# parsaeskandar/pangenome-index

Measured on AMD Instinct MI355X. Metric: find_mems reads/sec (150 bp batch), higher is better.
Workload: dtype u64

## Files before the change

pangenome-index_amd/csrc/pgx_batch.hip:

```cpp
#include <memory>
#include <string>
#include <thread>

#include "pgx_runtime_internal.hpp"

struct pgx_chunk { uint64_t r0, r1, slot_base, slots; };

struct pgx_batch {
    pgx_index *h = nullptr;
    pgx_device_image *dimg = nullptr;
    int device = 0;
    hipStream_t own = nullptr;
    hipStream_t side = nullptr;
    hipEvent_t ev_side[2] = {nullptr, nullptr};
    bool class_valid = false, class_ok = false;
    uint64_t side_reads_est = 0;
    uint64_t n_reads = 0, read_bytes = 0;
    HostBuf h_off[2];
    int h_off_cur = 0;
    const uint64_t *h_offsets() const { return h_off[h_off_cur].as<uint64_t>(); }
    std::vector<pgx_chunk> chunks;
    bool plan_valid = false, slot_off_valid = false;
    uint64_t slot_off_min_len = 0;
    uint64_t plan_min_len = 0, plan_budget = 0;
// ... 243 lines not shown
        HIPCHECK(hipGetLastError());
    }
    HIPCHECK(hipMemsetAsync((uint8_t *)b->reads.p + total, 0, 32, s));
    std::swap(b->offsets, b->fx_offs);
    HIPCHECK(hipMemcpyAsync(hb.p, b->offsets.p, (n_reads + 1) * 8, hipMemcpyDeviceToHost, s));
    HIPCHECK(hipStreamSynchronize(s));
    batch_reset_for_upload(b, n_reads, longest, total);
    *n_reads_out = n_reads;
}

extern "C" pgx_status pgx_batch_create(pgx_index *h, int device, const uint8_t *reads, const uint64_t *offsets,
                                       uint64_t n_reads, pgx_batch **out) {
    PGX_GUARD_BEGIN
    if (!h || !out || !offsets || (!reads && n_reads && offsets[n_reads] != offsets[0]))
        throw Error(PGX_ERR_ARG, "pgx_batch_create: null argument");
    if (!h->has_rank) throw Error(PGX_ERR_ARG, "pgx_batch_create: index opened without an r-index");
    *out = nullptr;
    pgx_device_image *dimg = device_image(h, device);
    ensure_lce(h, dimg);
    std::unique_ptr<pgx_batch, void (*)(pgx_batch *)> b(new pgx_batch(), batch_release);
    b->h = h;
    b->dimg = dimg;
    b->device = device;
    HIPCHECK(hipStreamCreateWithFlags(&b->own, hipStreamNonBlocking));
    batch_upload(b.get(), reads, offsets, n_reads);
    *out = b.release();
    return PGX_OK;
    PGX_GUARD_END
}

extern "C" pgx_status pgx_batch_upload(pgx_batch *b, const uint8_t *reads, const uint64_t *offsets, uint64_t n_reads) {
    PGX_GUARD_BEGIN
    RoctxRange range("pgx_batch_upload");
    if (!b || !offsets || (!reads && n_reads && offsets[n_reads] != offsets[0])) throw Error(PGX_ERR_ARG, "pgx_batch_upload: null argument");
    use_device(b->device);
    batch_upload(b, reads, offsets, n_reads);
    return PGX_OK;
    PGX_GUARD_END
}

extern "C" pgx_status pgx_batch_upload_packed(pgx_batch *b, const uint32_t *packed, const uint64_t *offsets, uint64_t n_reads, const uint64_t *side_ids,
                                              const uint8_t *side_bytes, uint64_t n_side) {
    PGX_GUARD_BEGIN
    RoctxRange range("pgx_batch_upload_packed");
    if (!b || !offsets || (!packed && n_reads && offsets[n_reads] != offsets[0]) || (n_side && (!side_ids || !side_bytes)))
        throw Error(PGX_ERR_ARG, "pgx_batch_upload_packed: null argument");
    use_device(b->device);
    batch_upload_packed(b, packed, offsets, n_reads, side_ids, side_bytes, n_side);
    return PGX_OK;
    PGX_GUARD_END
}

extern "C" pgx_status pgx_batch_upload_text(pgx_batch *b, const uint8_t *text, uint64_t n_bytes, uint32_t format, uint64_t *n_reads) {
    PGX_GUARD_BEGIN
    RoctxRange range("pgx_batch_upload_text");
    if (!b || !n_reads || (!text && n_bytes)) throw Error(PGX_ERR_ARG, "pgx_batch_upload_text: null argument");
    if (format > PGX_READS_FASTQ) throw Error(PGX_ERR_ARG, "pgx_batch_upload_text: unknown format " + std::to_string(format));
    use_device(b->device);
    batch_upload_text(b, text, n_bytes, format, n_reads);
    return PGX_OK;
    PGX_GUARD_END
}


struct RunKnobs {
    bool spec;
    bool arena;
    bool has_arena_cap;
    uint64_t arena_cap;
    uint64_t budget_slots;
    bool narrow;
    bool force_redo;
    bool pairs;
    bool side;
    bool packed;
    int coop;
    bool lce;
    bool has_wg_per_cu;
    int wg_per_cu;
    uint32_t heavy_ext;
    bool has_side_heavy_ext;
    uint32_t side_heavy_ext;
    bool debug_counters;
    bool fm_stats;
};

static RunKnobs read_run_knobs() {
    auto is_set = [](const char *name) { return std::getenv(name) != nullptr; };
    auto not_zero = [](const char *name) { const char *e = std::getenv(name); return !(e && e[0] == '0'); };
    RunKnobs k{};
    k.spec = not_zero("PGX_SPEC");
    k.arena = not_zero("PGX_SLOT_ARENA");
    if (const char *e = std::getenv("PGX_SLOT_ARENA_CAP")) { k.has_arena_cap = true; k.arena_cap = std::strtoull(e, nullptr, 10); }
    if (const char *e = std::getenv("PGX_SLOT_BUDGET_MB")) k.budget_slots = std::max<uint64_t>(1, std::strtoull(e, nullptr, 10)) * (1ull << 20) / sizeof(pgx_mem);
    k.narrow = not_zero("PGX_FM_NARROW");
    k.force_redo = is_set("PGX_FM_NARROW_FORCE_REDO");
    k.pairs = not_zero("PGX_FM_PAIRS");
    k.side = !is_set("PGX_FM_NO_SIDE");
    k.packed = not_zero("PGX_FM_PACKED");
    k.coop = -1;
    if (const char *e = std::getenv("PGX_FM_COOP")) k.coop = e[0] == '1';
    k.lce = not_zero("PGX_FM_LCE");
    if (const char *e = std::getenv("PGX_FM_WG_PER_CU")) { k.has_wg_per_cu = true; k.wg_per_cu = std::atoi(e); }
    k.heavy_ext = PGX_FM_HEAVY_EXT;
    if (const char *e = std::getenv("PGX_FM_HEAVY_EXT")) k.heavy_ext = (uint32_t)std::strtoul(e, nullptr, 10);
    if (const char *e = std::getenv("PGX_FM_SIDE_HEAVY_EXT")) { k.has_side_heavy_ext = true; k.side_heavy_ext = (uint32_t)std::strtoul(e, nullptr, 10); }
    k.debug_counters = is_set("PGX_DEBUG_COUNTERS");
    k.fm_stats = is_set("PGX_FM_STATS");
    return k;
}

static const void *find_mems_entry(bool in_lds, uint32_t kind, bool narrow, bool seeded) {
    using K = const void *;
    static const K tab[2][4][2][2] = {
        {{{(K)pgx_find_mems_kernel<false, 0, false, false>, nullptr}, {nullptr, nullptr}},
         {{(K)pgx_find_mems_kernel<false, 1, false, false>, (K)pgx_find_mems_kernel<false, 1, false, true>},
          {(K)pgx_find_mems_kernel<false, 1, true, false>, (K)pgx_find_mems_kernel<false, 1, true, true>}},
         {{(K)pgx_find_mems_kernel<false, 2, false, false>, (K)pgx_find_mems_kernel<false, 2, false, true>},
          {(K)pgx_find_mems_kernel<false, 2, true, false>, (K)pgx_find_mems_kernel<false, 2, true, true>}},
         {{(K)pgx_find_mems_kernel<false, 3, false, false>, (K)pgx_find_mems_kernel<false, 3, false, true>}, {nullptr, nullptr}}},
        {{{(K)pgx_find_mems_kernel<true, 0, false, false>, nullptr}, {nullptr, nullptr}},
         {{(K)pgx_find_mems_kernel<true, 1, false, false>, (K)pgx_find_mems_kernel<true, 1, false, true>},
          {(K)pgx_find_mems_kernel<true, 1, true, false>, (K)pgx_find_mems_kernel<true, 1, true, true>}},
         {{nullptr, nullptr}, {nullptr, nullptr}},
         {{nullptr, nullptr}, {nullptr, nullptr}}}};
    return kind < 4 ? tab[in_lds][kind][narrow][seeded] : nullptr;
}

static uint32_t find_mems_bits(bool in_lds, uint32_t kind, bool narrow, bool seeded) {
    return PGX_KERNELS_FM | (seeded ? PGX_KERNELS_FM_SEEDED : 0u) | (narrow ? PGX_KERNELS_FM_NARROW : 0u) | (kind << PGX_KERNELS_FM_KIND_SHIFT) | (in_lds ? PGX_KERNELS_FM_LDS : 0u);
}

static const void *find_mems_variant(bool in_lds, uint32_t kind, bool narrow, bool seeded, uint32_t &bits) {
    if (kind == 0) seeded = false;
    const void *f = find_mems_entry(in_lds, kind, narrow, seeded);
    if (!f) throw Error(PGX_ERR_UNSUPPORTED, "pgx_batch_run: no find_mems kernel for this image");
    bits = find_mems_bits(in_lds, kind, narrow, seeded);
    return f;
}

static const void *find_mems_pairs_entry(bool wide, bool packed, bool coop, bool s64, bool lce) {
    using K = const void *;
    static const K plain[2][2] = {
        {(K)pgx_find_mems_pairs_kernel<true, false, false, false, false, false>, (K)pgx_find_mems_pairs_kernel<true, false, false, false, true, false>},
        {(K)pgx_find_mems_pairs_kernel<true, true, false, false, false, false>, (K)pgx_find_mems_pairs_kernel<true, true, false, false, true, false>}};
    static const K pack[2][2][2] = {
        {{(K)pgx_find_mems_pairs_kernel<true, false, true, false, false, false>, (K)pgx_find_mems_pairs_kernel<true, false, true, false, true, false>},
         {(K)pgx_find_mems_pairs_kernel<true, false, true, true, false, false>, (K)pgx_find_mems_pairs_kernel<true, false, true, true, true, false>}},
        {{(K)pgx_find_mems_pairs_kernel<true, true, true, false, false, false>, (K)pgx_find_mems_pairs_kernel<true, true, true, false, true, false>},
         {(K)pgx_find_mems_pairs_kernel<true, true, true, true, false, false>, (K)pgx_find_mems_pairs_kernel<true, true, true, true, true, false>}}};
    static const K with_lce[2] = {(K)pgx_find_mems_pairs_kernel<true, false, true, false, false, true>, (K)pgx_find_mems_pairs_kernel<true, false, true, false, true, true>};
    if (lce) return (wide || !packed || coop) ? nullptr : with_lce[s64];
    if (!packed) return coop ? nullptr : plain[wide][s64];
    return pack[wide][coop][s64];
}

static uint32_t find_mems_pairs_bits(bool wide, bool packed, bool coop, bool s64, bool lce) {
    return PGX_KERNELS_PAIRS | (s64 ? PGX_KERNELS_PAIRS_S64 : 0u) | (coop ? PGX_KERNELS_PAIRS_COOP : 0u) | (packed ? PGX_KERNELS_PAIRS_PACKED : 0u) |
           (wide ? PGX_KERNELS_PAIRS_WIDE : 0u) | (lce ? PGX_KERNELS_PAIRS_LCE : 0u);
}

static const void *find_mems_pairs_variant(bool wide, bool packed, bool coop, bool s64, bool lce, uint32_t &bits) {
    const void *f = find_mems_pairs_entry(wide, packed, coop, s64, lce);
    if (!f && lce) throw Error(PGX_ERR_UNSUPPORTED, "pgx_batch_run: no LCE pairs kernel for this image");
    if (!f) throw Error(PGX_ERR_UNSUPPORTED, "pgx_batch_run: no cooperative pairs kernel without the packed reads");
    bits = find_mems_pairs_bits(wide, packed, coop, s64, lce);
    return f;
}

extern "C" uint32_t pgx_kernel_variants(uint32_t *out, uint32_t cap) {
    uint32_t n = 0;
    auto put = [&](uint32_t bits) { if (out && n < cap) out[n] = bits; n++; };
    for (int c = 0; c < 32; c++) {
        const bool in_lds = c & 16, narrow = c & 2, seeded = c & 1;
        const uint32_t kind = (c >> 2) & 3;
        if (find_mems_entry(in_lds, kind, narrow, seeded)) put(find_mems_bits(in_lds, kind, narrow, seeded));
    }
    for (int c = 0; c < 32; c++) {
        const bool wide = c & 16, packed = c & 8, coop = c & 4, s64 = c & 2, lce = c & 1;
        if (find_mems_pairs_entry(wide, packed, coop, s64, lce)) put(find_mems_pairs_bits(wide, packed, coop, s64, lce));
    }
    return n;
}

struct RunCtx {
    pgx_batch *b;
    hipStream_t s;
    RunKnobs k;
    PgxDevImage img;
    uint64_t n, min_len, min_occ;
    bool want_tags;
    unsigned long long *ctr = nullptr;
    bool spec = false, arena_on = false;
    uint64_t cm_cap = 0;
    const void *kfn = nullptr, *kfn_wide = nullptr, *kfn_pairs = nullptr;
    uint32_t kfn_bits = 0, kfn_pairs_bits = 0;
    size_t pairs_lds = 0;
    int cus = 0;
    bool fresh_work = false, fresh_mark = false;
    uint64_t n_ext = 0;
    float ms_fm = 0, ms_cp = 0, ms_main = 0;
};

struct FmArgs {
    PgxDevImage img;
    const uint8_t *reads;
    const uint64_t *off, *slot_off;
    uint64_t n, min_len, min_occ, base, first;
    pgx_mem *slots;
    uint32_t *cnt;
    unsigned long long *next, *cur;
    uint32_t hext, hcap;
    pgx_heavy_item *hlist;
    unsigned long long *hcount;
    uint32_t *ovf;
    uint64_t ovf_cap;
};

static void record(pgx_batch *b, int i, hipStream_t s) {
    static const char *const stage[10] = {"pgx: run begins (classify, sizing)", "pgx: find_mems launches follow", "pgx: find_mems enqueued", "pgx: compaction enqueued",
                                          "pgx: tag locate enqueued", "pgx: tag gather enqueued", "pgx: tag sort/unique enqueued", "pgx: run enqueued", "pgx: main find_mems kernel enqueued",
                                          "pgx: per-upload passes enqueued"};
    if (roctx().on) roctx().mark(stage[i]);
    if (!b->timed) return;
    if (!b->ev[i]) HIPCHECK(hipEventCreate(&b->ev[i]));
    HIPCHECK(hipEventRecord(b->ev[i], s));
}

static unsigned find_mems_grid(const RunCtx &r, const void *kfn, size_t lds, bool few_suffice, uint64_t cn) {
    int wg = 0;
    HIPCHECK(hipOccupancyMaxActiveBlocksPerMultiprocessor(&wg, kfn, PGX_FM_THREADS, lds));
    if (wg < 1) wg = 1;
    if (r.k.has_wg_per_cu) {
        if (r.k.wg_per_cu >= 1 && r.k.wg_per_cu < wg) wg = r.k.wg_per_cu;
    } else if (few_suffice)
        wg = (int)std::min<uint64_t>((uint64_t)wg, std::max<uint64_t>(2, cn / (5ull * (uint64_t)r.cus * PGX_FM_THREADS)));
    return std::min(grid_for(cn, 64), (unsigned)(wg * r.cus));
}

static void plan_slots(RunCtx &r) {
    pgx_batch *b = r.b;
    const uint64_t n = r.n, min_len = r.min_len;
    b->slot_off.ensure((n + 1) * 8);
    if (!b->slot_off_valid || b->slot_off_min_len != min_len) {
        r.fresh_work = true;
        scan_excl(2, b->offsets.p, n, min_len, b->slot_off.as<uint64_t>(), b->scan_tmp, r.s);
        b->slot_off_valid = true;
        b->slot_off_min_len = min_len;
    }
    b->mem_count.ensure((n ? n : 1) * 4);
    b->mem_off.ensure((n + 1) * 8);
    uint64_t budget_slots = (16ull << 30) / sizeof(pgx_mem);
    {
        size_t mem_free = 0, mem_total = 0;
        if (hipMemGetInfo(&mem_free, &mem_total) == hipSuccess) budget_slots = std::max<uint64_t>(budget_slots, (uint64_t)(mem_total / 4) / sizeof(pgx_mem));
        else (void)hipGetLastError();
    }
    if (r.k.budget_slots) budget_slots = r.k.budget_slots;
    if (!b->plan_valid || b->plan_min_len != min_len || b->plan_budget != budget_slots) {
        b->chunks.clear();
        uint64_t r0 = 0, base = 0, acc = 0;
        if (n && b->read_bytes <= budget_slots) b->chunks.push_back({0, n, 0, std::max<uint64_t>(b->read_bytes, 1)});
        else {
            for (uint64_t i = 0; i < n; i++) {
                const uint64_t len = b->h_offsets()[i + 1] - b->h_offsets()[i];
                const uint64_t cap = len < min_len ? 0 : std::min<uint64_t>(len, len - min_len + 1);
                if (acc && acc + cap > budget_slots) { b->chunks.push_back({r0, i, base, acc}); r0 = i; base += acc; acc = 0; }
                acc += cap;
            }
            if (n) b->chunks.push_back({r0, n, base, acc});
        }
        b->plan_valid = true; b->plan_min_len = min_len; b->plan_budget = budget_slots;
    }
    uint64_t max_chunk_reads = 1;
    for (auto &c : b->chunks) max_chunk_reads = std::max(max_chunk_reads, c.r1 - c.r0);
    b->ovf_base.ensure(max_chunk_reads * 4);
// ... 114 lines not shown
    ovf_cap = arena_slots(r, c);
    for (int attempt = 0;; attempt++) {
        b->slots.ensure(((ovf_cap ? ovf_cap : c.slots) + 4 * cn) * sizeof(pgx_mem));
        if (ci || attempt) {
            HIPCHECK(hipMemsetAsync(r.ctr, 0, PGX_CTR_TAG0 * 8, s));
            HIPCHECK(hipMemsetAsync(r.ctr + PGX_CTR_ARENA0, 0, (PGX_CTR_ALL - PGX_CTR_ARENA0) * 8, s));
        }
        FmArgs a;
        a.img = r.img;
        a.reads = b->reads.as<uint8_t>();
        a.off = b->offsets.as<uint64_t>(); a.slot_off = b->slot_off.as<uint64_t>();
        a.n = c.r1; a.min_len = r.min_len; a.min_occ = r.min_occ; a.base = c.slot_base; a.first = c.r0;
        a.slots = b->slots.as<pgx_mem>();
        a.cnt = b->mem_count.as<uint32_t>();
        a.next = r.ctr; a.cur = r.ctr + PGX_CTR_CURSOR;
        a.hext = heavy_ext; a.hcap = PGX_FM_HEAVY_CAP;
        a.hlist = b->heavy_list.as<pgx_heavy_item>();
        a.hcount = r.ctr + PGX_CTR_HEAVY;
        a.ovf = b->ovf_base.as<uint32_t>() - c.r0;
        a.ovf_cap = ovf_cap;
        bool side_running = false;
        if (r.kfn_pairs) {
            const uint8_t *skip = nullptr;
            if (one_chunk && r.k.side) {
                if (!b->side) {
                    HIPCHECK(hipStreamCreateWithFlags(&b->side, hipStreamNonBlocking));
                    for (auto &e : b->ev_side) HIPCHECK(hipEventCreateWithFlags(&e, hipEventDisableTiming));
                }
                if (!b->class_valid) classify_reads(r, cn);
                record(b, 9, s); r.fresh_mark = true;
                if (b->class_ok) {
                    skip = b->read_flags.as<uint8_t>();
                    launch_side(r, a, kf, grid);
                    side_running = true;
                }
            }
            launch_pairs(r, a, skip, cn, grid);
        } else {
            const pgx_heavy_item *a_rlist = nullptr;
            const unsigned long long *a_rcount = nullptr;
            void *args[] = {&a.img, &a.reads, &a.off, &a.n, &a.min_len, &a.min_occ, &a.slot_off, &a.slots, &a.cnt, &a.next, &a.cur, &a.first, &a.base,
                            &a.hext, &a.hcap, &a.hlist, &a.hcount, &a_rlist, &a_rcount, &a.ovf, &a.ovf_cap};
            if (ci == 0 && attempt == 0) { record(b, 9, s); r.fresh_mark = true; }
            HIPCHECK(hipLaunchKernel(kf, dim3(grid), dim3(PGX_FM_THREADS), args, b->dimg->lds_bytes, s));
            b->timing.kernels |= r.kfn_bits | (kf != r.kfn ? PGX_KERNELS_FM_REDO : 0u);
        }
        record(b, 8, s);
        if (side_running) HIPCHECK(hipStreamWaitEvent(s, b->ev_side[1], 0));
        if (heavy_ext) {
            b->timing.kernels |= PGX_KERNELS_HEAVY;
            if (b->dimg->lds_bytes)
                hipLaunchKernelGGL(pgx_find_mems_heavy_kernel<true>, dim3(PGX_FM_HEAVY_GRID), dim3(256), b->dimg->lds_bytes, s, r.img, a.reads, a.off,
                                   r.min_len, r.min_occ, a.slot_off, c.slot_base, a.slots, a.cnt, r.ctr, (const pgx_heavy_item *)a.hlist,
                                   (const unsigned long long *)a.hcount, (uint32_t)PGX_FM_HEAVY_CAP, b->heavy_scratch.as<PgxHeavyResult>(), c.r0, cn, a.ovf, a.ovf_cap);
            else
                hipLaunchKernelGGL(pgx_find_mems_heavy_kernel<false>, dim3(PGX_FM_HEAVY_GRID), dim3(256), 0, s, r.img, a.reads, a.off, r.min_len, r.min_occ,
                                   a.slot_off, c.slot_base, a.slots, a.cnt, r.ctr, (const pgx_heavy_item *)a.hlist,
                                   (const unsigned long long *)a.hcount, (uint32_t)PGX_FM_HEAVY_CAP, b->heavy_scratch.as<PgxHeavyResult>(), c.r0, cn, a.ovf, a.ovf_cap);
        }
        if (ovf_cap) hipLaunchKernelGGL(pgx_arena_demand_kernel, dim3(1), dim3(PGX_ARENA_SUBS), 0, s, r.ctr);
        HIPCHECK(hipGetLastError());
        b->timing.find_mems_launches++;
        record(b, 2, s);
        scan_excl(0, b->mem_count.as<uint32_t>() + c.r0, cn, 0, local, b->scan_tmp, s, reinterpret_cast<uint64_t *>(r.ctr + PGX_CTR_MEMS));
        if (r.spec) return r.cm_cap;
        unsigned long long cc[16];
        read_scalars(cc, r.ctr, sizeof cc, s);
        if (ovf_cap) b->last_ovf_used = cc[PGX_CTR_OVF_TOP];
        if (ovf_cap && cc[PGX_CTR_OVF_ABORT]) { ovf_cap = 0; continue; }
        const bool forced = attempt == 0 && kf != r.kfn_wide && r.k.force_redo;
        if ((cc[PGX_CTR_OVF32] || forced) && kf != r.kfn_wide) { kf = r.kfn_wide; continue; }
        r.n_ext += cc[PGX_CTR_EXT];
        b->timing.heavy_reads += (uint32_t)std::min<unsigned long long>(cc[PGX_CTR_HEAVY], PGX_FM_HEAVY_CAP);
        b->timing.pairs_other_steps += (uint32_t)cc[PGX_CTR_REDO];
        return cc[PGX_CTR_MEMS];
    }
}

static void compact_chunk(RunCtx &r, const pgx_chunk &c, uint64_t cm, uint64_t mem_base, uint64_t ovf_cap) {
    pgx_batch *b = r.b;
    hipStream_t s = r.s;
    const uint64_t cn = c.r1 - c.r0;
    b->mems.ensure_keep((mem_base + cm ? mem_base + cm : 1) * sizeof(pgx_mem), mem_base * sizeof(pgx_mem));
    hipLaunchKernelGGL(pgx_compact_mems_kernel, dim3(grid_for(cn, 256)), dim3(256), 0, s, c.r0, cn, b->slot_off.as<uint64_t>(),
                       c.slot_base, b->slots.as<pgx_mem>(), b->mem_count.as<uint32_t>(), (const uint64_t *)(b->mem_off.as<uint64_t>() + c.r0), mem_base,
                       b->mems.as<pgx_mem>(), r.spec ? r.cm_cap : ~0ull, reinterpret_cast<uint64_t *>(r.ctr + PGX_CTR_ABORT),
                       (const uint32_t *)(b->ovf_base.as<uint32_t>() - c.r0), ovf_cap);
    HIPCHECK(hipGetLastError());
    record(b, 3, s);
    if (b->timed && b->chunks.size() > 1) {
        HIPCHECK(hipStreamSynchronize(s));
        float t1 = 0, t2 = 0, t3 = 0;
        HIPCHECK(hipEventElapsedTime(&t1, b->ev[1], b->ev[2]));
        HIPCHECK(hipEventElapsedTime(&t2, b->ev[2], b->ev[3]));
        HIPCHECK(hipEventElapsedTime(&t3, b->ev[1], b->ev[8]));
        r.ms_fm += t1; r.ms_cp += t2; r.ms_main += t3;
    }
}

static bool read_back(RunCtx &r, bool &force_worst) {
    pgx_batch *b = r.b;
    const size_t n_chunks = b->chunks.size();
    unsigned long long cnt[PGX_CTR_SLOTS];
    read_scalars(cnt, b->counters.p, sizeof cnt, r.s);
    if (r.spec) {
        b->spec_runs++;
        if (cnt[PGX_CTR_OVF_ABORT]) { force_worst = true; b->last_ovf_used = cnt[PGX_CTR_OVF_TOP]; }
        if (r.k.debug_counters)
            std::fprintf(stderr, "[pgx] speculative run: abort flags %llu, 32-bit overflow %llu, arena overflow %llu (top %llu), MEMs %llu of capacity %llu\n", cnt[PGX_CTR_ABORT], cnt[PGX_CTR_OVF32],
                         cnt[PGX_CTR_OVF_ABORT], cnt[PGX_CTR_OVF_TOP], cnt[PGX_CTR_MEMS], (unsigned long long)r.cm_cap);
        if (cnt[PGX_CTR_ABORT] || cnt[PGX_CTR_OVF32] || cnt[PGX_CTR_OVF_ABORT] || cnt[PGX_CTR_MEMS] > r.cm_cap) { b->spec_fallbacks++; b->ran_tags = false; return false; }
        b->last_ovf_used = cnt[PGX_CTR_OVF_TOP];
        b->n_mems = cnt[PGX_CTR_MEMS];
        r.n_ext = cnt[PGX_CTR_EXT];
        b->timing.heavy_reads = (uint32_t)std::min<unsigned long long>(cnt[PGX_CTR_HEAVY], PGX_FM_HEAVY_CAP);
        b->timing.pairs_other_steps = (uint32_t)cnt[PGX_CTR_REDO];
        if (r.want_tags) {
            TagWork &w = b->tw;
            const unsigned long long *tc = cnt + PGX_CTR_TAG0;
            w.last_big = tc[0]; w.last_large = tc[1]; w.last_largest = tc[2]; w.last_G = tc[3]; w.last_small = tc[5];
            w.last_rep = tc[6]; w.last_dup = tc[7]; w.last_P = tc[8];
            w.n_positions = tc[8];
            b->n_positions = tc[8];
        }
    }
    if (r.kfn_pairs) {
        b->timing.main_lines = cnt[PGX_CTR_PAIRS_LINES]; b->timing.main_seed_loads = cnt[PGX_CTR_PAIRS_SEEDS];
        b->timing.other_lines = cnt[PGX_CTR_FM_LINES]; b->timing.other_seed_loads = cnt[PGX_CTR_FM_SEEDS];
        b->timing.two_step_trips = cnt[PGX_CTR_PAIRS_TWO];
    } else { b->timing.main_lines = cnt[PGX_CTR_FM_LINES]; b->timing.main_seed_loads = cnt[PGX_CTR_FM_SEEDS]; }
    b->last_mems = b->n_mems;
    b->shape_valid = true; b->shape_reads = r.n; b->shape_min_len = r.min_len; b->shape_min_occ = r.min_occ; b->shape_tags = r.want_tags;
    if (cnt[PGX_CTR_ST_TRIPS] && r.k.fm_stats)
        std::fprintf(stderr, "[pgx] find_mems wave trips %llu, live lane-trips %llu (%.1f%% of lanes), longest wave %llu trips, extensions %llu\n", cnt[PGX_CTR_ST_TRIPS],
                     cnt[PGX_CTR_ST_LIVE], 100.0 * (double)cnt[PGX_CTR_ST_LIVE] / (64.0 * (double)cnt[PGX_CTR_ST_TRIPS]), cnt[PGX_CTR_ST_LONGEST], cnt[PGX_CTR_EXT]);
    if (cnt[PGX_CTR_ST_PAIR_TRIPS] && r.k.fm_stats)
        std::fprintf(stderr, "[pgx] pairs kernel wave trips %llu, live lane-trips %llu (%.1f%%), with two extensions %llu, waiting for a second block %llu, fresh %llu, extensions through the other image %llu\n",
                     cnt[PGX_CTR_ST_PAIR_TRIPS], cnt[PGX_CTR_ST_PAIR_LIVE], 100.0 * (double)cnt[PGX_CTR_ST_PAIR_LIVE] / (64.0 * (double)cnt[PGX_CTR_ST_PAIR_TRIPS]),
                     cnt[PGX_CTR_PAIRS_TWO], cnt[PGX_CTR_ST_PAIR_WAIT], cnt[PGX_CTR_ST_PAIR_FRESH], cnt[PGX_CTR_REDO]);
    if (cnt[PGX_CTR_ST_PAIR_T_TOTAL] && r.k.fm_stats)
        std::fprintf(stderr, "[pgx] pairs kernel clock ticks: %.1f%% of the waves' time in the refill loop (%llu of %llu), %llu trips with a refill round; waiting for the seed entry %.1f%%, then for the block line %.1f%%\n",
                     100.0 * (double)cnt[PGX_CTR_ST_PAIR_T_REFILL] / (double)cnt[PGX_CTR_ST_PAIR_T_TOTAL], cnt[PGX_CTR_ST_PAIR_T_REFILL], cnt[PGX_CTR_ST_PAIR_T_TOTAL], cnt[PGX_CTR_ST_PAIR_REFILLS],
                     100.0 * (double)cnt[PGX_CTR_ST_PAIR_T_SEED] / (double)cnt[PGX_CTR_ST_PAIR_T_TOTAL], 100.0 * (double)cnt[PGX_CTR_ST_PAIR_T_LINE] / (double)cnt[PGX_CTR_ST_PAIR_T_TOTAL]);
    if (r.k.debug_counters)
        std::fprintf(stderr, "[pgx] counters: extensions %llu tag overflows %llu heavy %llu other-image steps %llu lines %llu + %llu seeds %llu + %llu\n", cnt[PGX_CTR_EXT], cnt[PGX_CTR_TAG_OVERFLOW],
                     cnt[PGX_CTR_HEAVY], cnt[PGX_CTR_REDO], cnt[PGX_CTR_PAIRS_LINES], cnt[PGX_CTR_FM_LINES], cnt[PGX_CTR_PAIRS_SEEDS], cnt[PGX_CTR_FM_SEEDS]);
    b->n_ext = r.n_ext;
    b->n_tag_overflow = cnt[PGX_CTR_TAG_OVERFLOW];
    if (b->timed) {
        auto el = [&](int a, int c) { float ms = 0; HIPCHECK(hipEventElapsedTime(&ms, b->ev[a], b->ev[c])); return ms; };
        b->timing.ms_find_mems = n_chunks > 1 ? r.ms_fm : el(1, 2);
        b->timing.ms_find_mems_main = n_chunks > 1 ? r.ms_main : (r.n ? el(1, 8) : 0.0f);
        b->timing.ms_compact = n_chunks > 1 ? r.ms_cp : el(2, 3);
        if (r.want_tags) {
            b->timing.ms_tag_locate = el(3, 4);
            b->timing.ms_tag_gather = el(4, 5);
            b->timing.ms_tag_sort = el(5, 6);
        }
        b->timing.ms_total = el(0, 7);
        if (r.fresh_work) b->timing.ms_per_upload = b->ms_upload_passes + (r.fresh_mark ? el(0, 9) : 0.0f);
    }
    if (r.fresh_work) b->ms_upload_passes = 0;
    return true;
}

static bool run_pass(RunCtx &r, bool may_speculate, bool &force_worst) {
    pgx_batch *b = r.b;
    hipStream_t s = r.s;
    b->n_mems = b->n_positions = b->n_ext = b->n_tag_overflow = 0;
    std::memset(&b->timing, 0, sizeof b->timing);
    r.fresh_work = r.fresh_mark = false;
    r.n_ext = 0;
    r.ms_fm = r.ms_cp = r.ms_main = 0;
    b->counters.ensure(PGX_CTR_ALL * 8);
    HIPCHECK(hipMemsetAsync(b->counters.p, 0, PGX_CTR_ALL * 8, s));
    r.ctr = b->counters.as<unsigned long long>();

    record(b, 0, s);
    plan_slots(r);
    const std::vector<pgx_chunk> &chunks = b->chunks;
    r.arena_on = r.k.arena && !force_worst;
    r.kfn = r.kfn_wide = r.kfn_pairs = nullptr;
    r.cus = 0;
    if (r.n) choose_kernels(r);
    if (r.k.heavy_ext) {
        b->heavy_list.ensure((size_t)PGX_FM_HEAVY_CAP * sizeof(pgx_heavy_item));
        b->heavy_scratch.ensure((size_t)PGX_FM_HEAVY_GRID * PGX_FM_HEAVY_MAXLEN * sizeof(PgxHeavyResult));
    }
    r.spec = may_speculate && chunks.size() == 1 && b->shape_valid && b->shape_reads == r.n && b->shape_min_len == r.min_len && b->shape_min_occ == r.min_occ &&
             b->shape_tags == r.want_tags && (!r.want_tags || (b->tw.have_last && b->tw.last_largest <= PGX_SORT_WG_LDS_CAP)) && r.k.spec && !r.k.force_redo;
    r.cm_cap = with_slack(b->last_mems);
    uint64_t mem_base = 0;
    for (size_t ci = 0; ci < chunks.size(); ci++) {
        record(b, 1, s);
        uint64_t ovf_cap = 0;
        const uint64_t cm = find_mems_chunk(r, ci, ovf_cap);
        compact_chunk(r, chunks[ci], cm, mem_base, ovf_cap);
        mem_base += cm;
    }
    b->n_mems = mem_base;
    if (!r.kfn_pairs) b->timing.pairs_reads = 0u;
    else if (!b->timing.pairs_reads) b->timing.pairs_reads = 1u;
    b->timing.seed_depth = (r.img.seed_k != 0 && r.min_len >= r.img.seed_k && r.img.dense) ? r.img.seed_k : 0u;
    if (chunks.size() != 1) {
        if (chunks.empty()) { record(b, 1, s); record(b, 2, s); }
        scan_excl(0, b->mem_count.p, r.n, 0, b->mem_off.as<uint64_t>(), b->scan_tmp, s);
        b->mems.ensure_keep((b->n_mems ? b->n_mems : 1) * sizeof(pgx_mem), b->n_mems * sizeof(pgx_mem));
        record(b, 3, s);
    }
    record(b, 3, s);
    if (r.want_tags) {
        tag_pipeline(r.img, b->mems.as<pgx_mem>(), nullptr, nullptr, b->n_mems, b->tw, r.ctr + PGX_CTR_TAG_OVERFLOW, r.ctr + PGX_CTR_TAG0, s,
                     [&](int stage) { record(b, 4 + stage, s); }, r.spec, reinterpret_cast<const uint64_t *>(r.ctr + PGX_CTR_MEMS),
                     reinterpret_cast<uint64_t *>(r.ctr + PGX_CTR_ABORT));
        b->n_positions = b->tw.n_positions;
        b->ran_tags = true;
    }
    record(b, 7, s);
    return read_back(r, force_worst);
}

extern "C" pgx_status pgx_batch_run(pgx_batch *b, uint64_t min_len, uint64_t min_occ, uint32_t flags, void *stream) {
    PGX_GUARD_BEGIN
    RoctxRange range("pgx_batch_run");
    if (!b) throw Error(PGX_ERR_ARG, "pgx_batch_run: null batch");
    use_device(b->device);
    RunCtx r{b, stream ? (hipStream_t)stream : b->own, read_run_knobs(), b->dimg->img, b->n_reads, min_len, min_occ, (flags & PGX_RUN_TAGS) != 0};
    PgxDevImage &img = r.img;
    if (img.seed_k_main && min_len < img.seed_k_main && img.seed_k_small && min_len >= img.seed_k_small) { img.seed = img.seed_small; img.seed_k = img.seed_k_small; }
    if (r.want_tags && !b->h->has_tags) throw Error(PGX_ERR_ARG, "pgx_batch_run: PGX_RUN_TAGS without a tag array");
    b->timed = (flags & PGX_RUN_TIMING) != 0;
    b->ran = false;
    b->ran_tags = false;
    b->lw.valid = false;
    b->n_mems = b->n_positions = b->n_ext = b->n_tag_overflow = 0;
    std::memset(&b->timing, 0, sizeof b->timing);
    bool force_worst = false;
    if (!run_pass(r, true, force_worst)) run_pass(r, false, force_worst);
    b->ran = true;
    return PGX_OK;
    PGX_GUARD_END
}

extern "C" pgx_status pgx_batch_device_result(pgx_batch *b, pgx_device_result *out) {
    PGX_GUARD_BEGIN
    if (!b || !out || !b->ran) throw Error(PGX_ERR_ARG, "pgx_batch_device_result: batch has not been run");
    std::memset(out, 0, sizeof *out);
    out->n_reads = b->n_reads;
    out->n_mems = b->n_mems;
    out->mem_offsets = b->mem_off.as<uint64_t>();
    out->mems = b->mems.as<pgx_mem>();
    if (b->ran_tags) {
        out->n_positions = b->n_positions;
        out->tag_run_counts = b->tw.run_nums.as<uint64_t>();
        out->pos_offsets = b->tw.pos_off.as<uint64_t>();
        out->positions = b->tw.positions.as<uint64_t>();
    }
    return PGX_OK;
    PGX_GUARD_END
}

extern "C" pgx_status pgx_batch_counts(pgx_batch *b, uint64_t *n_mems, uint64_t *n_positions, uint64_t *n_extensions) {
    PGX_GUARD_BEGIN
    if (!b || !b->ran) throw Error(PGX_ERR_ARG, "pgx_batch_counts: batch has not been run");
    if (n_mems) *n_mems = b->n_mems;
    if (n_positions) *n_positions = b->n_positions;
    if (n_extensions) *n_extensions = b->n_ext;
    return PGX_OK;
    PGX_GUARD_END
}

extern "C" pgx_status pgx_batch_spec_stats(pgx_batch *b, uint32_t *speculative_runs, uint32_t *fallbacks) {
    PGX_GUARD_BEGIN
    if (!b) throw Error(PGX_ERR_ARG, "pgx_batch_spec_stats: null batch");
    if (speculative_runs) *speculative_runs = b->spec_runs;
    if (fallbacks) *fallbacks = b->spec_fallbacks;
    return PGX_OK;
    PGX_GUARD_END
}

extern "C" pgx_status pgx_batch_timing(pgx_batch *b, pgx_timing *out) {
    PGX_GUARD_BEGIN
    if (!b || !out || !b->ran) throw Error(PGX_ERR_ARG, "pgx_batch_timing: batch has not been run");
    if (!b->timed) throw Error(PGX_ERR_ARG, "pgx_batch_timing: run without PGX_RUN_TIMING");
    *out = b->timing;
    return PGX_OK;
    PGX_GUARD_END
}

extern "C" pgx_status pgx_batch_result(pgx_batch *b, pgx_result *out) {
    PGX_GUARD_BEGIN
    RoctxRange range("pgx_batch_result");
    if (!b || !out || !b->ran) throw Error(PGX_ERR_ARG, "pgx_batch_result: batch has not been run");
    use_device(b->device);
    const uint64_t n = b->n_reads, m = b->n_mems;
    b->h_mem_off.ensure((n + 1) * 8);
// ... 303 lines not shown
```

pangenome-index_amd/csrc/pgx_device.h:

```cpp
#pragma once

#include <hip/hip_runtime.h>
#include <stdint.h>

#include "../../include/pgx.h"
#include "pgx_image.h"

enum PgxCounterSlot {
    PGX_CTR_EXT = 0,
    PGX_CTR_TAG_OVERFLOW = 1,
    PGX_CTR_CURSOR = 5,
    PGX_CTR_HEAVY = 8,
    PGX_CTR_OVF32 = 9,
    PGX_CTR_MEMS = 10,
    PGX_CTR_REDO = 11,
    PGX_CTR_REDO_CURSOR = 12,
    PGX_CTR_SIDE_CURSOR = 13,
    PGX_CTR_OVF_TOP = 14,
    PGX_CTR_OVF_ABORT = 15,
    PGX_CTR_TAG0 = 16,
    PGX_CTR_ABORT = 30,
    PGX_CTR_PAIRS_LINES = 32,
    PGX_CTR_PAIRS_SEEDS = 33,
    PGX_CTR_FM_LINES = 34,
// ... 34 lines not shown
    uint32_t dir_shift;
    uint32_t excl_mask;
    uint32_t tag_dir_shift;
    uint32_t dense;
    const uint32_t *exc;
    uint32_t seed_k;
    const uint4 *seed;
    uint32_t seed_end_k;
    const uint4 *seed_end;
    uint32_t seed_k_main, seed_k_small;
    const uint4 *seed_main, *seed_small;
    const uint4 *pairs;
    const uint4 *first_ext;
    uint32_t pair_runs;
    const uint64_t *sbase2, *pbase;
    uint32_t d2_sb_shift, pairs_sb_shift, n_sb2, n_sbp;
    uint32_t wide;
    uint32_t pairs_stride;
    const uint32_t *lce_sa;
    const uint32_t *lce_text;
    const uint32_t *lce_flags;
    const uint8_t *lce_lcp;
    uint32_t lce_max;
    uint32_t refill_min;
};
#define PGX_LCP_CAP 254u
#define PGX_LCP_UNKNOWN 255u
#define PGX_SEED_UNUSABLE 255u
#define PGX_SEED_MAX_K 16
#define PGX_SEED_SMALL_K 10

struct pgx_heavy_item {
    uint64_t rid;
    uint32_t x, nm;
};
struct PgxHeavyResult {
    pgx_mem mem;
    uint32_t next_x, n_ext, has_mem, pad;
};
#define PGX_FM_HEAVY_EXT 2048u
#define PGX_FM_SIDE_HEAVY_EXT 2048u
#define PGX_FM_HEAVY_MAXLEN 4096u
#define PGX_FM_HEAVY_CAP 8192u
#define PGX_FM_HEAVY_GRID 64u
template <bool LDS_IMAGE>
__global__ void pgx_find_mems_heavy_kernel(PgxDevImage img, const uint8_t *reads, const uint64_t *offsets, uint64_t min_len, uint64_t min_occ,
                                           const uint64_t *slot_off, uint64_t slot_base, pgx_mem *slots, uint32_t *mem_count,
                                           unsigned long long *n_ext_total, const pgx_heavy_item *heavy_list,
                                           const unsigned long long *heavy_count, uint32_t heavy_cap, PgxHeavyResult *scratch, uint64_t chunk_first,
                                           uint64_t chunk_reads, uint32_t *ovf_base, uint64_t ovf_cap);

__global__ void pgx_seed_build_kernel(PgxDevImage img, const uint4 *src, uint4 *dst, uint32_t level, uint64_t n_dst, uint64_t limit, int end_table);
template <bool LDS_IMAGE, int DENSE, bool NARROW, bool SEED>
__global__ void pgx_find_mems_kernel(PgxDevImage img, const uint8_t *reads, const uint64_t *offsets, uint64_t n_reads,
                                     uint64_t min_len, uint64_t min_occ, const uint64_t *slot_off, pgx_mem *slots,
                                     uint32_t *mem_count, unsigned long long *n_ext_total, unsigned long long *cursor, uint64_t first_read,
                                     uint64_t slot_base, uint32_t heavy_ext, uint32_t heavy_cap, pgx_heavy_item *heavy_list, unsigned long long *heavy_count,
                                     const pgx_heavy_item *rid_list, const unsigned long long *rid_count, uint32_t *ovf_base, uint64_t ovf_cap);
template <bool SEED, bool WIDE, bool PACKED, bool COOP, bool S64, bool LCE>
__global__ void pgx_find_mems_pairs_kernel(PgxDevImage img, const uint8_t *reads, const uint64_t *offsets, uint64_t n_reads,
                                           uint64_t min_len, uint64_t min_occ, const uint64_t *slot_off, pgx_mem *slots,
                                           uint32_t *mem_count, unsigned long long *n_ext_total, unsigned long long *cursor, uint64_t first_read,
                                           uint64_t slot_base, uint32_t heavy_ext, uint32_t heavy_cap, pgx_heavy_item *heavy_list, unsigned long long *heavy_count,
                                           const uint8_t *skip, const uint32_t *packed, uint32_t pk_words,
                                           uint32_t *ovf_base, uint64_t ovf_cap);
__global__ void pgx_bad_chunks_kernel(const uint8_t *reads, uint64_t n_bytes, uint64_t *chunks, unsigned long long *count, uint64_t cap, uint32_t *packed);
__global__ void pgx_unpack_reads_kernel(const uint32_t *packed, uint64_t n_chunks, uint8_t *reads);
__global__ void pgx_side_reads_kernel(uint8_t *reads, const uint64_t *offsets, const uint64_t *side_ids, const uint64_t *side_off, const uint8_t *side_bytes, uint64_t n_side,
                                      uint8_t *flags, pgx_heavy_item *list, unsigned long long *count);
__global__ void pgx_classify_reads_kernel(const uint8_t *reads, const uint64_t *offsets, uint64_t n_reads, const uint64_t *chunks, const unsigned long long *n_chunks,
                                          uint64_t cap, uint32_t *flag_words, pgx_heavy_item *list, unsigned long long *count);
__global__ void pgx_first_ext_kernel(PgxDevImage img, uint4 *out);
__global__ void pgx_rank_kernel(PgxDevImage img, const uint64_t *pos, uint64_t n, int true_codes, uint64_t *out);
template <bool LOOP, bool MULHI> __global__ void pgx_rank_probe_kernel(PgxDevImage img, const uint64_t *pos, uint64_t n, uint64_t *out);
template <bool LDS_IMAGE>
__global__ void pgx_extend_kernel(PgxDevImage img, const pgx_biint *in, const uint8_t *sym, const uint8_t *forward, uint64_t n,
                                  pgx_biint *out);
template <bool LDS_IMAGE>
__global__ void pgx_count_kernel(PgxDevImage img, const uint8_t *reads, const uint64_t *offsets, uint64_t n_reads, pgx_range *out);
__global__ void pgx_fmf_kernel(PgxDevImage img, const uint8_t *reads, const uint64_t *offsets, const uint64_t *read_of, const uint64_t *xs, uint64_t n,
                               uint64_t min_len, uint64_t min_occ, PgxHeavyResult *out);
__global__ void pgx_lf_kernel(PgxDevImage img, const pgx_range *in, const uint8_t *sym, uint64_t n, pgx_range *out);
__global__ void pgx_scan_partial_kernel(int mode, const void *in, uint64_t n, uint64_t min_len, uint64_t *block_sums, const uint64_t *n_dev);
template <int MODE>
__global__ void pgx_scan_onepass_kernel(const void *in, uint64_t n, uint64_t min_len, uint64_t *out, uint64_t *total_out, const uint64_t *n_dev,
                                        unsigned long long *state, uint32_t epoch);
__global__ void pgx_scan_sums_kernel(uint64_t *block_sums, uint64_t nb);
__global__ void pgx_scan_apply_kernel(int mode, const void *in, uint64_t n, uint64_t min_len, const uint64_t *block_sums,
                                      uint64_t nb, uint64_t *out, uint64_t *total_out, int raw_sums, const uint64_t *n_dev);
__global__ void pgx_compact_mems_kernel(uint64_t first_read, uint64_t n_reads, const uint64_t *slot_off, uint64_t slot_base,
                                        const pgx_mem *slots, const uint32_t *mem_count, const uint64_t *local_off,
                                        uint64_t mem_base, pgx_mem *mems, uint64_t cap_mems, uint64_t *abort, const uint32_t *ovf_base, uint64_t ovf_cap);
__global__ void pgx_tag_pair_kernel(const uint64_t *tstart, const uint64_t *tvals, uint64_t n_runs, uint64_t n_items, ulonglong2 *out);
__global__ void pgx_tag_bucket_kernel(const uint64_t *tstart, const uint64_t *tvals, uint64_t n_runs, uint64_t n_items, uint32_t shift, uint64_t n_buckets, uint4 *out);
#define PGX_TAG_LOCATE_THREADS 1024
#define PGX_SORT_LDS_CAP 2048
#define PGX_TAG_SMALL 16
#define PGX_SORT_WG_LDS_CAP 16384

__global__ void pgx_tag_locate_kernel(PgxDevImage img, const pgx_mem *mems, const uint64_t *qstart, const uint64_t *qend,
                                      uint64_t n, const uint64_t *n_dev, const uint64_t *abort, uint64_t *run_nums, uint64_t *first_item, uint64_t *need,
                                      uint64_t *big_list, uint64_t *large_list, unsigned long long *n_big, unsigned long long *n_large, uint64_t *single,
                                      uint64_t *ucount, unsigned long long *n_overflow, uint64_t *small_list, unsigned long long *n_small);
__global__ void pgx_tag_small_kernel(PgxDevImage img, const uint64_t *list, uint64_t n, const uint64_t *n_dev, const uint64_t *abort, const uint64_t *run_nums,
                                     const uint64_t *first_item, const uint64_t *seg_off, uint64_t *buf, uint64_t *ucount, unsigned long long *n_overflow);
__global__ void pgx_tag_gather_kernel(PgxDevImage img, const uint64_t *list, uint64_t n_list, const uint64_t *n_dev, const uint64_t *abort,
                                      const uint64_t *run_nums, const uint64_t *first_item, const uint64_t *seg_off, uint64_t *buf,
                                      unsigned long long *n_overflow);
__global__ void pgx_tag_sort_unique_kernel(const uint64_t *list, uint64_t n_list, const uint64_t *n_dev, const uint64_t *abort, const uint64_t *run_nums,
                                           const uint64_t *seg_off, uint64_t *buf, uint64_t *ucount);
__global__ void pgx_tag_sort_large_kernel(const uint64_t *list, uint64_t n_list, const uint64_t *n_dev, const uint64_t *abort, const uint64_t *run_nums,
                                          const uint64_t *seg_off, uint64_t *buf, uint64_t *scratch, const uint64_t *scratch_off, uint64_t *ucount);
__global__ void pgx_tag_dedup_kernel(const uint64_t *list, uint64_t n_list, const uint64_t *n_dev, const uint64_t *abort, const uint64_t *first_item,
                                     const uint64_t *run_nums, unsigned long long *table, uint64_t table_mask, uint64_t *reps, unsigned long long *n_rep,
                                     uint64_t *pairs, unsigned long long *n_dup);
__global__ void pgx_tag_copy_dups_kernel(const uint64_t *pairs, uint64_t n_pairs, const uint64_t *n_dev, const uint64_t *abort, uint64_t n_tag_items,
                                         const uint64_t *first_item, const uint64_t *run_nums, uint64_t *seg_off, uint64_t *buf, uint64_t *ucount,
                                         unsigned long long *n_overflow);
__global__ void pgx_tag_compact_kernel(const uint64_t *list, uint64_t n, const uint64_t *n_dev, const uint64_t *abort, const uint64_t *ucount,
                                       const uint64_t *seg_off, const uint64_t *buf, const uint64_t *pos_off, uint64_t *positions, uint64_t max_count);
__global__ void pgx_tag_compact_single_kernel(uint64_t n, const uint64_t *n_dev, const uint64_t *abort, const uint64_t *run_nums, const uint64_t *single,
                                              const uint64_t *pos_off, uint64_t *positions);
__global__ void pgx_tag_compact_list_kernel(const uint64_t *list, uint64_t n_list, const uint64_t *n_dev, const uint64_t *abort, const uint64_t *ucount,
                                            const uint64_t *seg_off, const uint64_t *buf, const uint64_t *pos_off, uint64_t *positions, uint64_t max_count);
__global__ void pgx_spec_check_kernel(const uint64_t *v0, uint64_t c0, const uint64_t *v1, uint64_t c1, const uint64_t *v2, uint64_t c2,
                                      const uint64_t *v3, uint64_t c3, uint64_t *abort);
#define PGX_TAG_COMPACT_SMALL 256

struct PgxLocImage {
    const uint64_t *rstart, *rsamp;
    const uint32_t *rdir;
    const uint64_t *lpos, *lnext;
    const uint32_t *ldir;
    uint64_t n, n_runs, n_last, max_length, rdir_entries, ldir_entries;
    uint32_t rdir_shift, ldir_shift;
};
__global__ void pgx_locate_next_kernel(PgxLocImage loc, const uint64_t *prev, uint64_t n, uint64_t *out);
__global__ void pgx_lce_seqlen_kernel(const uint64_t *sa, uint64_t n_seq, uint64_t max_length, unsigned long long *seq_len);
__global__ void pgx_lce_scatter_kernel(const uint64_t *sa, uint64_t n, uint64_t max_length, const uint64_t *seq_start, uint64_t n_seq, uint64_t c1, uint64_t c2, uint64_t c3,
                                       uint64_t c4, uint64_t c5, uint32_t *sa32, uint8_t *text8, unsigned long long *bad);
__global__ void pgx_lce_pack_kernel(const uint8_t *text8, uint64_t n, uint64_t n_words, uint32_t *text32, uint32_t *flags);
__global__ void pgx_lce_lcp_kernel(const uint32_t *sa32, const uint32_t *text32, const uint32_t *flags, uint64_t n, uint8_t *lcp);
__global__ void pgx_lce_rc_check_kernel(const uint8_t *text8, const uint64_t *seq_start, uint64_t n_seq, uint64_t n, unsigned long long *bad);
__global__ void pgx_locate_plan_kernel(PgxLocImage loc, const uint64_t *qs, const uint64_t *qe, uint64_t n, uint64_t *run0,
                                       uint64_t *n_pieces);
__global__ void pgx_locate_walk_kernel(PgxLocImage loc, const uint64_t *qs, const uint64_t *qe, uint64_t n_queries,
                                       const uint64_t *run0, const uint64_t *piece_off, uint64_t n_pieces, const uint64_t *val_off,
                                       uint64_t val_base, int seq_ids, uint64_t *out);

#define PGX_ML_SPAN 4096
#define PGX_ML_WIN 1024
__global__ void pgx_ml_plan_kernel(const pgx_mem *mems, uint64_t n, uint64_t bwt_n, uint64_t max_occ, uint64_t *cnt, uint64_t *qs, uint64_t *qe,
                                   unsigned long long *n_not_located);
__global__ void pgx_ml_cut_kernel(const uint64_t *off, uint64_t n, uint64_t m0, uint64_t budget, uint64_t *out);
__global__ void pgx_ml_gather_kernel(const pgx_mem *mems, const uint64_t *off, uint64_t m0, uint64_t m1, uint64_t o_first, uint64_t nv,
                                     const uint32_t *sa32, uint64_t bwt_n, const uint64_t *seq_start, uint64_t n_seq, uint64_t max_length,
                                     int seq_ids, uint64_t *out);
__global__ void pgx_ml_classify_kernel(const uint64_t *cnt, const uint64_t *off, uint64_t np, uint64_t *seg, uint64_t *wave_list,
                                       uint64_t *wg_list, uint64_t *need, uint64_t *ucount, unsigned long long *ctr);
#define PGX_ML_SET_WORDS_MAX 64
#define PGX_ML_SET_BATCH 8
#define PGX_ML_SET_WIN 2048
__global__ void pgx_ml_sets_kernel(const pgx_mem *mems, const uint64_t *off, uint64_t m0, uint64_t m1, uint64_t o_first, uint64_t nv,
                                   const uint32_t *sa32, uint64_t bwt_n, const uint64_t *seq_start, uint64_t n_seq, uint32_t W,
                                   unsigned long long *sets);
__global__ void pgx_ml_sets_ids_kernel(const uint64_t *off, uint64_t m0, uint64_t m1, uint64_t o_first, uint64_t nv, const uint64_t *ids, uint32_t W,
                                       unsigned long long *sets);
__global__ void pgx_ml_set_count_kernel(const unsigned long long *sets, uint64_t np, uint32_t W, uint32_t Wp, uint64_t *ucount);
__global__ void pgx_ml_set_expand_kernel(const unsigned long long *sets, uint64_t np, uint32_t W, const uint64_t *uloc, uint64_t *out);
__global__ void pgx_ml_stride_kernel(uint64_t *out, uint64_t n, uint64_t stride);

struct PgxLitImage {
    const uint64_t *bstart, *cum, *runs;
    const uint32_t *roff;
    const uint32_t *code_of, *cslot_of;
    uint64_t C[8];
    uint64_t n, n_blocks;
};
__global__ void pgx_lit_count_kernel(PgxLitImage lit, const uint8_t *reads, const uint64_t *offsets, const pgx_range *in, const uint8_t *sym,
                                     uint64_t n, pgx_range *out);

__global__ void pgx_mt_file_of_kernel(const uint64_t *da, uint64_t n, uint64_t n_seq, const uint32_t *seq_to_file, uint32_t n_files,
                                      uint8_t *file_of, unsigned long long *n_bad);
__global__ void pgx_mt_expand_kernel(const uint64_t *start, const uint64_t *val, uint64_t n_runs, uint64_t *out);
__global__ void pgx_mt_gather_kernel(const uint8_t *file_of, uint32_t f, const uint64_t *rank, const uint64_t *expanded, uint64_t total,
                                     uint64_t n, uint64_t *tags);
// ... 33 lines not shown
```

pangenome-index_amd/csrc/pgx_kernels.hip:

```cpp
#include <hip/hip_runtime.h>
#include <stdint.h>

#include <type_traits>

#include "pgx_device.h"

template <bool LDS_IMAGE>
__device__ __forceinline__ uint32_t pgx_find_block(const PgxDevImage &img, const uint64_t *__restrict__ lds_dir,
                                                   const uint16_t *__restrict__ lds_blow, uint64_t pos) {
    const uint64_t di = pos >> img.dir_shift;
    const uint64_t e = LDS_IMAGE ? lds_dir[di] : img.dir[di];
    const uint32_t lowp = (uint32_t)pos & ((1u << img.dir_shift) - 1u);
    uint32_t lo = (uint32_t)e;
    const uint32_t cnt = (uint32_t)(e >> 32) & 0xFFu;
    if (cnt <= 2) {
        const uint32_t l0 = (uint32_t)(e >> 40) & 0xFFFu, l1 = (uint32_t)(e >> 52);
        return lo - 1u + ((cnt >= 1 && l0 <= lowp) ? 1u : 0u) + ((cnt >= 2 && l1 <= lowp) ? 1u : 0u);
    }
    uint32_t hi = cnt < 255 ? lo + cnt : (uint32_t)(LDS_IMAGE ? lds_dir[di + 1] : img.dir[di + 1]);
    while (lo < hi) {
        const uint32_t mid = (lo + hi) >> 1;
        const uint32_t v = LDS_IMAGE ? lds_blow[mid] : img.blow[mid];
        if (v <= lowp) lo = mid + 1; else hi = mid;
    }
// ... 359 lines not shown
        k = 0; kp = 0; s = 0;
        return;
    }
    const uint64_t nk = A0 + s_C[PGX_EXT_V(e)], nq = kq + dB;
    s = A1 - A0;
    k = fwd ? nq : nk;
    kp = fwd ? nk : nq;
}

template <bool LDS_IMAGE>
__device__ __forceinline__ void pgx_stage_tables(const PgxDevImage &img, uint32_t *s_ext, uint64_t *s_C, uint4 *lds_blocks,
                                                 uint64_t *lds_dir, uint16_t *lds_blow) {
    for (uint32_t i = threadIdx.x; i < 512; i += blockDim.x) s_ext[i] = img.consts->ext_tab[i];
    if (threadIdx.x < 8) s_C[threadIdx.x] = img.consts->C[threadIdx.x];
    if (LDS_IMAGE) {
        const uint32_t nb4 = img.n_blocks * 4;
        for (uint32_t i = threadIdx.x; i < nb4; i += blockDim.x) lds_blocks[img.dense ? (i >> 2) * PGX_DENSE_LDS_U4 + (i & 3u) : i] = img.blocks[i];
        if (!img.dense)
            for (uint64_t i = threadIdx.x; i < img.dir_entries; i += blockDim.x) lds_dir[i] = img.dir[i];
        if (!img.dense)
            for (uint32_t i = threadIdx.x; i < img.n_blocks; i += blockDim.x) lds_blow[i] = img.blow[i];
    }
    __syncthreads();
}

#define PGX_LDS_CARVE(img)                                                                   \
    extern __shared__ __align__(16) unsigned char pgx_dyn_lds[];                              \
    uint4 *lds_blocks = reinterpret_cast<uint4 *>(pgx_dyn_lds);                               \
    uint64_t *lds_dir = reinterpret_cast<uint64_t *>(pgx_dyn_lds + (size_t)(img).n_blocks * PGX_BLOCK_BYTES);    \
    uint16_t *lds_blow = reinterpret_cast<uint16_t *>(pgx_dyn_lds + (size_t)(img).n_blocks * PGX_BLOCK_BYTES + (img).dir_entries * 8)

__device__ __forceinline__ uint32_t pgx_seed_codes(uint64_t x, uint64_t &bad) {
    const uint64_t c = (x >> 1) & 0x0303030303030303ull;
    const uint64_t b0 = c & 0x0101010101010101ull, b1 = (c >> 1) & 0x0101010101010101ull;
    const uint64_t recon = 0x4141414141414141ull + 2 * (b0 & ~b1) + 0x13 * (b1 & ~b0) + 6 * (b0 & b1);
    bad = x ^ recon;
    uint64_t t = (c | (c >> 6)) & 0x000F000F000F000Full;
    t = (t | (t >> 12)) & 0x000000FF000000FFull;
    t = (t | (t >> 24)) & 0xFFFFull;
    return (uint32_t)t;
}
__device__ __forceinline__ bool pgx_seed_index(uint64_t lo, uint64_t hi, uint32_t K, uint32_t &idx) {
    uint64_t badlo, badhi;
    const uint32_t ilo = pgx_seed_codes(lo, badlo), ihi = pgx_seed_codes(hi, badhi);
    const uint32_t nlo = K < 8u ? K : 8u, nhi = K > 8u ? K - 8u : 0u;
    const uint64_t mlo = nlo == 8u ? ~0ull : ((1ull << (8u * nlo)) - 1ull), mhi = nhi == 8u ? ~0ull : ((1ull << (8u * nhi)) - 1ull);
    idx = (ilo & ((1u << (2u * nlo)) - 1u)) | ((ihi & ((1u << (2u * nhi)) - 1u)) << 16);
    return ((badlo & mlo) | (badhi & mhi)) == 0ull;
}

__global__ void __launch_bounds__(256)
pgx_seed_build_kernel(PgxDevImage img, const uint4 *__restrict__ src, uint4 *__restrict__ dst, uint32_t level, uint64_t n_dst, uint64_t limit, int end_table) {
    __shared__ uint32_t s_ext[512];
    __shared__ uint64_t s_C[8];
    pgx_stage_tables<false>(img, s_ext, s_C, nullptr, nullptr, nullptr);
  for (uint64_t i = (uint64_t)blockIdx.x * blockDim.x + threadIdx.x; i < n_dst; i += (uint64_t)gridDim.x * blockDim.x) {
    uint64_t k = 0, kp = 0, s = img.n;
    uint32_t depth = 0;
    const uint32_t base_depth = end_table ? 1u : 0u;
    if (end_table && !level) {
        pgx_extend<false>(img, nullptr, nullptr, nullptr, s_ext, s_C, k, kp, s, 0u, false);
        if (s == 0) { k = 0; kp = 0; depth = 1u; }
    }
    if (level) {
        const uint4 e = src[i >> 2];
        k = (uint64_t)e.x | ((uint64_t)(e.w & 0xFFu) << 32);
        kp = (uint64_t)e.y | ((uint64_t)((e.w >> 8) & 0xFFu) << 32);
        s = (uint64_t)e.z | ((uint64_t)((e.w >> 16) & 0xFFu) << 32);
        depth = e.w >> 24;
    }
    if (s != 0) {
        const uint32_t byte = (0x47544341u >> (8u * (uint32_t)(i & 3))) & 0xFFu;
        pgx_extend<false>(img, nullptr, nullptr, nullptr, s_ext, s_C, k, kp, s, byte, false);
        if (s == 0) { k = 0; kp = 0; depth = level + 1 + base_depth; }
        else if (k >= limit || kp >= limit || k + s >= limit || kp + s >= limit || k + s < k || kp + s < kp) { k = 0; kp = 0; s = 0; depth = PGX_SEED_UNUSABLE; }
    }
    uint4 o;
    o.x = (uint32_t)k; o.y = (uint32_t)kp; o.z = (uint32_t)s;
    o.w = (uint32_t)(k >> 32) | ((uint32_t)(kp >> 32) << 8) | ((uint32_t)(s >> 32) << 16) | (depth << 24);
    dst[i] = o;
  }
}

#define PGX_FAST_SLOTS 4u
#ifndef PGX_PAIRS_PACKED_WAVES
#define PGX_PAIRS_PACKED_WAVES 5
#endif
#define PGX_PK_GROUP 12u
__device__ __forceinline__ uint64_t pgx_slot_index(uint64_t read_in_chunk, uint64_t chunk_reads, uint64_t slot, uint32_t nm) {
    return nm < PGX_FAST_SLOTS ? (uint64_t)nm * chunk_reads + read_in_chunk : chunk_reads * PGX_FAST_SLOTS + slot + nm;
}
__device__ __forceinline__ uint64_t pgx_slot_extent(const uint64_t *__restrict__ slot_off, uint64_t slot_base, uint32_t *__restrict__ ovf_base, uint64_t ovf_cap,
                                                    unsigned long long *__restrict__ ctr, uint64_t rid, uint32_t nm, int32_t len, int32_t x, uint64_t min_len) {
    if (!ovf_cap) return slot_off[rid] - slot_base;
    if (nm == PGX_FAST_SLOTS) {
        const int64_t ml = min_len ? (int64_t)min_len : 1;
        const int64_t left = (int64_t)len - ml - (int64_t)x + 1;
        const unsigned long long ext = left > 0 ? (unsigned long long)left : 1ull;
        const uint32_t sub = (uint32_t)rid & (PGX_ARENA_SUBS - 1u);
        const uint64_t sub_cap = ovf_cap / PGX_ARENA_SUBS;
        unsigned long long at = atomicAdd(ctr + PGX_CTR_ARENA0 + 16u * sub, ext);
        if (at + ext > sub_cap) { ctr[PGX_CTR_OVF_ABORT] = 1ull; at = 0ull; }
        at += (unsigned long long)sub * sub_cap;
        ovf_base[rid] = (uint32_t)at;
        return at - PGX_FAST_SLOTS;
    }
    return (uint64_t)ovf_base[rid] - PGX_FAST_SLOTS;
}

#define PGX_FM_BATCH (LDS_IMAGE ? 128u : 32u)
template <bool LDS_IMAGE, int DENSE, bool NARROW, bool SEED>
__global__ void __launch_bounds__(PGX_FM_THREADS, DENSE == 0 ? 3 : PGX_FM_WAVES_PER_SIMD)
pgx_find_mems_kernel(PgxDevImage img, const uint8_t *__restrict__ reads, const uint64_t *__restrict__ offsets,
                     uint64_t n_reads, uint64_t min_len, uint64_t min_occ, const uint64_t *__restrict__ slot_off,
                     pgx_mem *__restrict__ slots, uint32_t *__restrict__ mem_count, unsigned long long *__restrict__ n_ext_total,
                     unsigned long long *__restrict__ cursor, uint64_t first_read, uint64_t slot_base, uint32_t heavy_ext, uint32_t heavy_cap,
                     pgx_heavy_item *__restrict__ heavy_list, unsigned long long *__restrict__ heavy_count,
                     const pgx_heavy_item *__restrict__ rid_list, const unsigned long long *__restrict__ rid_count, uint32_t *__restrict__ ovf_base, uint64_t ovf_cap) {
    __shared__ uint32_t s_ext[512];
    __shared__ uint64_t s_C[8];
    __shared__ uint64_t s_sb[DENSE == 3 ? PGX_SB_MAX * 8 : 1];
    PGX_LDS_CARVE(img);
    if (DENSE == 3) for (uint32_t i = threadIdx.x; i < img.n_sb2 * 8u; i += blockDim.x) s_sb[i] = img.sbase2[i];
    pgx_stage_tables<LDS_IMAGE>(img, s_ext, s_C, lds_blocks, lds_dir, lds_blow);
    const uint64_t chunk_first = first_read, chunk_reads = n_reads - first_read;
    if (rid_list) { first_read = 0; n_reads = *rid_count; }

    static_assert(!NARROW || DENSE, "the 32-bit state exists for the dense image only");
    static_assert(!SEED || DENSE, "k-mer seeds exist for the dense images");
    static_assert(DENSE < 2 || !LDS_IMAGE, "the dense2 image is never staged in LDS");
    static_assert(DENSE != 3 || !NARROW, "the wide dense2 image is walked in 64 bits");
    typedef typename std::conditional<NARROW, uint32_t, uint64_t>::type pos_t;
    const int lane = threadIdx.x & 63;
    const pos_t n = (pos_t)img.n;
    uint64_t rid = 0, base = 0;
    int32_t len = 0, x = 0, j = 0;
    pos_t k = 0, kp = 0, s = 0, Jk = 0, Js = 0;
    uint32_t nm = 0, next = 0, next0 = 0;
    int ph = 0;
    uint64_t win = 0, win_hi = 0, win2 = 0, win3 = 0, win_at = ~0ull;
    pos_t A0 = 0, B0 = 0;
    bool pend = false;
    uint32_t fresh = 0;
    bool ovf = false;
    uint64_t rnext = 0, rend = 0;
    bool exhausted = false;
    unsigned long long ln_blk = 0, ln_seed = 0;
#ifdef PGX_FM_STATS
    unsigned long long st_trips = 0, st_live = 0;
#endif

    auto begin = [&]() __attribute__((always_inline)) {
        if (x >= len || (uint64_t)(len - x) < min_len) { ph = 0; mem_count[rid] = nm; return; }
        if (heavy_ext && next - next0 >= heavy_ext && len <= (int32_t)PGX_FM_HEAVY_MAXLEN) {
            const unsigned long long at = atomicAdd(heavy_count, 1ull);
            if (at < (unsigned long long)heavy_cap) {
                pgx_heavy_item it;
                it.rid = rid; it.x = (uint32_t)x; it.nm = nm;
                heavy_list[at] = it;
                ph = 0;
                return;
            }
        }
        k = 0; kp = 0; s = n;
        if (min_len == 0) {
            Jk = 0; Js = n; j = x; ph = 2;
        } else {
            j = x + (int32_t)min_len - 1; ph = 1;
            fresh = 1u;
        }
    };
    uint32_t restart = 0;
    auto emit = [&]() __attribute__((always_inline)) {
        pgx_mem m;
// ... 1107 lines not shown
            uint32_t nm = it.nm;
            unsigned long long ne = 0;
            int32_t x = x0;
            while (x < len && (uint64_t)(len - x) >= min_len) {
                const PgxHeavyResult r = res[x - x0];
                ne += r.n_ext;
                if (r.has_mem) {
                    const uint64_t slot = nm < PGX_FAST_SLOTS ? 0ull : pgx_slot_extent(slot_off, slot_base, ovf_base, ovf_cap, n_ext_total, it.rid, nm, len, x, min_len);
                    slots[pgx_slot_index(it.rid - chunk_first, chunk_reads, slot, nm)] = r.mem; nm++;
                }
                x = (int32_t)r.next_x;
            }
            mem_count[it.rid] = nm;
            atomicAdd(n_ext_total, ne);
        }
        __syncthreads();
    }
}
template __global__ void pgx_find_mems_heavy_kernel<false>(PgxDevImage, const uint8_t *, const uint64_t *, uint64_t, uint64_t, const uint64_t *, uint64_t,
                                                           pgx_mem *, uint32_t *, unsigned long long *, const pgx_heavy_item *,
                                                           const unsigned long long *, uint32_t, PgxHeavyResult *, uint64_t, uint64_t, uint32_t *, uint64_t);
template __global__ void pgx_find_mems_heavy_kernel<true>(PgxDevImage, const uint8_t *, const uint64_t *, uint64_t, uint64_t, const uint64_t *, uint64_t,
                                                          pgx_mem *, uint32_t *, unsigned long long *, const pgx_heavy_item *,
                                                          const unsigned long long *, uint32_t, PgxHeavyResult *, uint64_t, uint64_t, uint32_t *, uint64_t);

__global__ void __launch_bounds__(256)
pgx_rank_kernel(PgxDevImage img, const uint64_t *__restrict__ pos, uint64_t n, int true_codes, uint64_t *__restrict__ out) {
    const uint64_t t = (uint64_t)blockIdx.x * blockDim.x + threadIdx.x;
    if (t >= 6 * n) return;
    const uint64_t i = t / 6;
    const uint32_t sl = (uint32_t)(t - 6 * i);
    const uint32_t sigma = img.consts->sigma;
    uint64_t A = 0, B;
    if (true_codes) pgx_rank_ab<false>(img, nullptr, nullptr, nullptr, pos[i], sl, 0, A, B);
    else if (sl < sigma) pgx_rank_ab<false>(img, nullptr, nullptr, nullptr, pos[i], img.consts->slot_code[sl], 0, A, B);
    out[t] = A;
}
template <bool LOOP, bool MULHI>
__global__ void __launch_bounds__(256)
pgx_rank_probe_kernel(PgxDevImage img, const uint64_t *__restrict__ pos, uint64_t n, uint64_t *__restrict__ out) {
    const uint64_t t = (uint64_t)blockIdx.x * blockDim.x + threadIdx.x;
    if (LOOP) {
        if (t >= n) return;
        for (uint32_t sl = 0; sl < 6; sl++) {
            uint64_t A = 0, B;
            const uint64_t p = pos[t] > img.n ? img.n : pos[t];
            pgx_dense2w_rank<MULHI>(img, p, sl, 0, A, B);
            out[t * 6 + sl] = A;
        }
    } else {
        if (t >= 6 * n) return;
        const uint64_t i = t / 6;
        uint64_t A = 0, B;
        const uint64_t p = pos[i] > img.n ? img.n : pos[i];
        pgx_dense2w_rank<MULHI>(img, p, (uint32_t)(t - 6 * i), 0, A, B);
        out[t] = A;
    }
}
template __global__ void pgx_rank_probe_kernel<true, true>(PgxDevImage, const uint64_t *, uint64_t, uint64_t *);
template __global__ void pgx_rank_probe_kernel<true, false>(PgxDevImage, const uint64_t *, uint64_t, uint64_t *);
template __global__ void pgx_rank_probe_kernel<false, true>(PgxDevImage, const uint64_t *, uint64_t, uint64_t *);

template <bool LDS_IMAGE>
__global__ void __launch_bounds__(256)
pgx_extend_kernel(PgxDevImage img, const pgx_biint *__restrict__ in, const uint8_t *__restrict__ sym,
                  const uint8_t *__restrict__ forward, uint64_t n, pgx_biint *__restrict__ out) {
    __shared__ uint32_t s_ext[512];
    __shared__ uint64_t s_C[8];
    PGX_LDS_CARVE(img);
    pgx_stage_tables<LDS_IMAGE>(img, s_ext, s_C, lds_blocks, lds_dir, lds_blow);
    const uint64_t i = (uint64_t)blockIdx.x * blockDim.x + threadIdx.x;
    if (i >= n) return;
    uint64_t k = in[i].forward, kp = in[i].reverse, s = (uint64_t)in[i].size;
    pgx_extend<LDS_IMAGE>(img, lds_blocks, lds_dir, lds_blow, s_ext, s_C, k, kp, s, sym[i], forward[i] != 0);
    pgx_biint o;
    o.forward = k; o.reverse = kp; o.size = (int64_t)s;
    out[i] = o;
}
template __global__ void pgx_extend_kernel<false>(PgxDevImage, const pgx_biint *, const uint8_t *, const uint8_t *, uint64_t, pgx_biint *);
template __global__ void pgx_extend_kernel<true>(PgxDevImage, const pgx_biint *, const uint8_t *, const uint8_t *, uint64_t, pgx_biint *);

__device__ __forceinline__ uint64_t pgx_scan_load(int mode, const void *in, uint64_t i, uint64_t min_len) {
    if (mode == 0) return ((const uint32_t *)in)[i];
    if (mode == 1) return ((const uint64_t *)in)[i];
    if (mode == 3) return ((const uint8_t *)in)[i] == (uint8_t)min_len ? 1u : 0u;
    if (mode == 4) return ((const uint8_t *)in)[i];
    if (mode == 5) { const uint64_t v = ((const uint64_t *)in)[i]; return v == 1 ? 0 : v; }
    const uint64_t *off = (const uint64_t *)in;
    const uint64_t len = off[i + 1] - off[i];
    if (len < min_len) return 0;
    const uint64_t c = len - min_len + 1;
    return c < len ? c : len;
}

__device__ __forceinline__ uint64_t pgx_block_excl_scan(uint64_t v, uint64_t *s_wave, uint64_t &block_total) {
    const int lane = threadIdx.x & 63, w = threadIdx.x >> 6;
    uint64_t inc = v;
#pragma unroll
    for (int off = 1; off < 64; off <<= 1) {
        const uint64_t t = __shfl_up(inc, off, 64);
        if (lane >= off) inc += t;
    }
    if (lane == 63) s_wave[w] = inc;
    __syncthreads();
    uint64_t wbase = 0, tot = 0;
#pragma unroll
    for (int i = 0; i < 4; i++) {
        if (i < w) wbase += s_wave[i];
        tot += s_wave[i];
    }
    block_total = tot;
    __syncthreads();
    return wbase + inc - v;
}

#define PGX_SCAN_ITEMS 8
__global__ void __launch_bounds__(256)
pgx_scan_partial_kernel(int mode, const void *in, uint64_t n_cap, uint64_t min_len, uint64_t *__restrict__ block_sums, const uint64_t *__restrict__ n_dev) {
    __shared__ uint64_t s_wave[4];
    const uint64_t n = n_dev ? (*n_dev < n_cap ? *n_dev : n_cap) : n_cap;
    const uint64_t b0 = (uint64_t)blockIdx.x * 256 * PGX_SCAN_ITEMS;
    uint64_t v = 0;
    for (int t = 0; t < PGX_SCAN_ITEMS; t++) {
        const uint64_t i = b0 + (uint64_t)threadIdx.x * PGX_SCAN_ITEMS + t;
        if (i < n) v += pgx_scan_load(mode, in, i, min_len);
    }
    uint64_t tot;
    (void)pgx_block_excl_scan(v, s_wave, tot);
    if (threadIdx.x == 0) block_sums[blockIdx.x] = tot;
}

__global__ void __launch_bounds__(256) pgx_scan_sums_kernel(uint64_t *block_sums, uint64_t nb) {
    __shared__ uint64_t s_wave[4];
    uint64_t carry = 0;
    for (uint64_t b0 = 0; b0 < nb; b0 += 256) {
        const uint64_t i = b0 + threadIdx.x;
        const uint64_t v = i < nb ? block_sums[i] : 0;
        uint64_t tot;
        const uint64_t ex = pgx_block_excl_scan(v, s_wave, tot);
        if (i < nb) block_sums[i] = carry + ex;
        carry += tot;
    }
    if (threadIdx.x == 0) block_sums[nb] = carry;
}

__global__ void __launch_bounds__(256)
pgx_scan_apply_kernel(int mode, const void *in, uint64_t n_cap, uint64_t min_len, const uint64_t *__restrict__ block_sums,
                      uint64_t nb, uint64_t *__restrict__ out, uint64_t *__restrict__ total_out, int raw_sums, const uint64_t *__restrict__ n_dev) {
    __shared__ uint64_t s_wave[4];
    const uint64_t n = n_dev ? (*n_dev < n_cap ? *n_dev : n_cap) : n_cap;
    const uint64_t b0 = (uint64_t)blockIdx.x * 256 * PGX_SCAN_ITEMS;
    uint64_t base, grand = 0;
    if (raw_sums) {
        uint64_t part = 0, all = 0;
        for (uint64_t i = threadIdx.x; i < nb; i += 256) {
            const uint64_t t = block_sums[i];
            part += i < blockIdx.x ? t : 0;
            all += t;
        }
        uint64_t tot;
        (void)pgx_block_excl_scan(part, s_wave, tot);
        base = tot;
        if (blockIdx.x == 0) { (void)pgx_block_excl_scan(all, s_wave, tot); grand = tot; }
    } else {
        base = block_sums[blockIdx.x];
        grand = block_sums[nb];
    }
    uint64_t vals[PGX_SCAN_ITEMS], v = 0;
    for (int t = 0; t < PGX_SCAN_ITEMS; t++) {
        const uint64_t i = b0 + (uint64_t)threadIdx.x * PGX_SCAN_ITEMS + t;
        vals[t] = i < n ? pgx_scan_load(mode, in, i, min_len) : 0;
        v += vals[t];
    }
    uint64_t tot;
    uint64_t ex = base + pgx_block_excl_scan(v, s_wave, tot);
    for (int t = 0; t < PGX_SCAN_ITEMS; t++) {
        const uint64_t i = b0 + (uint64_t)threadIdx.x * PGX_SCAN_ITEMS + t;
        if (i < n) out[i] = ex;
        ex += vals[t];
    }
    if (blockIdx.x == 0 && threadIdx.x == 0) {
        out[n] = grand;
        if (total_out) *total_out = grand;
    }
}

#define PGX_SCAN1_ROUNDS 16
template <int MODE>
__global__ void __launch_bounds__(256)
pgx_scan_onepass_kernel(const void *in, uint64_t n_cap, uint64_t min_len, uint64_t *__restrict__ out, uint64_t *__restrict__ total_out,
                        const uint64_t *__restrict__ n_dev, unsigned long long *__restrict__ state, uint32_t epoch) {
    constexpr int mode = MODE;
    __shared__ uint64_t s_wave[4];
    __shared__ uint64_t s_prefix;
    __shared__ uint32_t s_tile;
    const uint64_t n = n_dev ? (*n_dev < n_cap ? *n_dev : n_cap) : n_cap;
    if (threadIdx.x == 0) s_tile = atomicAdd(reinterpret_cast<uint32_t *>(state), 1u);
    __syncthreads();
    const uint32_t tile = s_tile;
    const uint32_t last_tile = n ? (uint32_t)((n - 1) / (256u * PGX_SCAN1_ROUNDS)) : 0u;
    if (tile > last_tile) {
        if (tile == gridDim.x - 1 && threadIdx.x == 0) __hip_atomic_store(reinterpret_cast<uint32_t *>(state), 0u, __ATOMIC_RELAXED, __HIP_MEMORY_SCOPE_AGENT);
        return;
    }
    const int lane = threadIdx.x & 63, w = threadIdx.x >> 6;
    const uint64_t b0 = (uint64_t)tile * (256u * PGX_SCAN1_ROUNDS) + (uint64_t)w * (64u * PGX_SCAN1_ROUNDS);
    uint64_t x[PGX_SCAN1_ROUNDS], carry = 0;
#pragma unroll
    for (int r = 0; r < PGX_SCAN1_ROUNDS; r++) {
        const uint64_t i = b0 + (uint64_t)(r * 64 + lane);
        x[r] = i < n ? pgx_scan_load(mode, in, i, min_len) : 0;
    }
#pragma unroll
    for (int r = 0; r < PGX_SCAN1_ROUNDS; r++) {
        const uint64_t v = x[r];
        uint64_t inc = v;
#pragma unroll
        for (int off = 1; off < 64; off <<= 1) {
            const uint64_t t = __shfl_up(inc, off, 64);
            if (lane >= off) inc += t;
        }
        x[r] = carry + inc - v;
        carry += __shfl(inc, 63, 64);
    }
    if (lane == 0) s_wave[w] = carry;
    __syncthreads();
    uint64_t wbase = 0, tile_total = 0;
#pragma unroll
    for (int i = 0; i < 4; i++) { if (i < w) wbase += s_wave[i]; tile_total += s_wave[i]; }
    const unsigned long long ep = (unsigned long long)(epoch & 0x3FFFFu) << 46;
    const unsigned long long vmask = (1ull << 44) - 1ull;
    if (w == 0) {
        uint64_t prefix = 0;
        if (tile != 0) {
            if (lane == 0) __hip_atomic_store(state + 1 + tile, ep | (1ull << 44) | (tile_total & vmask), __ATOMIC_RELAXED, __HIP_MEMORY_SCOPE_AGENT);
            int64_t j = (int64_t)tile - 1;
            for (;;) {
                const int64_t idx = j - lane;
                unsigned long long word = ep | (2ull << 44);
                if (idx >= 0) word = __hip_atomic_load(state + 1 + idx, __ATOMIC_RELAXED, __HIP_MEMORY_SCOPE_AGENT);
                const uint32_t st = (word >> 46) == (ep >> 46) ? (uint32_t)(word >> 44) & 3u : 0u;
                const unsigned long long ready = __ballot(st != 0u), full = __ballot(st == 2u);
                const unsigned long long gap = ~ready;
                const int stop_gap = gap ? (int)__ffsll((long long)gap) - 1 : 64, stop_full = full ? (int)__ffsll((long long)full) - 1 : 64;
                if (stop_full < stop_gap) {
                    uint64_t v = lane <= stop_full ? (uint64_t)(word & vmask) : 0;
#pragma unroll
                    for (int off = 32; off > 0; off >>= 1) v += __shfl_down(v, off, 64);
                    prefix += __shfl(v, 0, 64);
                    break;
                }
                if (stop_gap == 64) {
                    uint64_t v = (uint64_t)(word & vmask);
#pragma unroll
                    for (int off = 32; off > 0; off >>= 1) v += __shfl_down(v, off, 64);
                    prefix += __shfl(v, 0, 64);
                    j -= 64;
                    continue;
                }
                __builtin_amdgcn_s_sleep(2);
            }
        }
        if (lane == 0) {
            __hip_atomic_store(state + 1 + tile, ep | (2ull << 44) | ((prefix + tile_total) & vmask), __ATOMIC_RELAXED, __HIP_MEMORY_SCOPE_AGENT);
            s_prefix = prefix;
        }
    }
    __syncthreads();
    const uint64_t P = s_prefix + wbase;
#pragma unroll
    for (int r = 0; r < PGX_SCAN1_ROUNDS; r++) {
        const uint64_t i = b0 + (uint64_t)(r * 64 + lane);
        if (i < n) out[i] = P + x[r];
    }
    if (tile == last_tile && threadIdx.x == 0) {
        const uint64_t grand = s_prefix + tile_total;
        out[n] = grand;
        if (total_out) *total_out = grand;
    }
    if (tile == gridDim.x - 1 && threadIdx.x == 0)
        __hip_atomic_store(reinterpret_cast<uint32_t *>(state), 0u, __ATOMIC_RELAXED, __HIP_MEMORY_SCOPE_AGENT);
}

#define PGX_SCAN1_INSTANTIATE(M) \
    template __global__ void pgx_scan_onepass_kernel<M>(const void *, uint64_t, uint64_t, uint64_t *, uint64_t *, const uint64_t *, unsigned long long *, uint32_t);
PGX_SCAN1_INSTANTIATE(0) PGX_SCAN1_INSTANTIATE(1) PGX_SCAN1_INSTANTIATE(2) PGX_SCAN1_INSTANTIATE(3) PGX_SCAN1_INSTANTIATE(4) PGX_SCAN1_INSTANTIATE(5)

__global__ void __launch_bounds__(256)
pgx_compact_mems_kernel(uint64_t first_read, uint64_t n_reads, const uint64_t *__restrict__ slot_off, uint64_t slot_base,
                        const pgx_mem *__restrict__ slots, const uint32_t *__restrict__ mem_count,
                        const uint64_t *__restrict__ local_off, uint64_t mem_base, pgx_mem *__restrict__ mems, uint64_t cap_mems,
                        uint64_t *__restrict__ abort, const uint32_t *__restrict__ ovf_base, uint64_t ovf_cap) {
    const uint64_t t = (uint64_t)blockIdx.x * blockDim.x + threadIdx.x;
    if (t >= n_reads) return;
    const uint64_t i = first_read + t;
    const uint32_t c = mem_count[i];
    const uint64_t src = c <= PGX_FAST_SLOTS ? 0ull : (ovf_cap ? (uint64_t)ovf_base[i] - PGX_FAST_SLOTS : slot_off[i] - slot_base), dst = mem_base + local_off[t];
    if (dst + c > cap_mems) {
        if (c && abort) atomicOr((unsigned long long *)abort, 16ull);
        return;
    }
    for (uint32_t u = 0; u < c; u++) mems[dst + u] = slots[pgx_slot_index(t, n_reads, src, u)];
}


template <bool LDS_IMAGE>
__global__ void __launch_bounds__(256)
pgx_count_kernel(PgxDevImage img, const uint8_t *__restrict__ reads, const uint64_t *__restrict__ offsets, uint64_t n_reads,
                 pgx_range *__restrict__ out) {
    __shared__ uint32_t s_cnt[256];
    __shared__ uint64_t s_C[8];
    PGX_LDS_CARVE(img);
    for (uint32_t i = threadIdx.x; i < 256; i += blockDim.x) s_cnt[i] = img.consts->cnt_tab[i];
    if (threadIdx.x < 8) s_C[threadIdx.x] = img.consts->C[threadIdx.x];
    if (LDS_IMAGE) {
        const uint32_t nb4 = img.n_blocks * 4;
        for (uint32_t i = threadIdx.x; i < nb4; i += blockDim.x) lds_blocks[img.dense ? (i >> 2) * PGX_DENSE_LDS_U4 + (i & 3u) : i] = img.blocks[i];
        if (!img.dense)
            for (uint64_t i = threadIdx.x; i < img.dir_entries; i += blockDim.x) lds_dir[i] = img.dir[i];
        if (!img.dense)
            for (uint32_t i = threadIdx.x; i < img.n_blocks; i += blockDim.x) lds_blow[i] = img.blow[i];
    }
    __syncthreads();
    const uint64_t rid = (uint64_t)blockIdx.x * blockDim.x + threadIdx.x;
    if (rid >= n_reads) return;
    const uint64_t base = offsets[rid], len = offsets[rid + 1] - base;
    uint64_t lo = 0, hi = img.n - 1;
    if (img.n == 0) { lo = 1; hi = 0; }
    for (uint64_t i = len; i > 0 && lo <= hi; i--) {
        const uint32_t e = s_cnt[reads[base + i - 1]];
        if (PGX_EXT_KILL(e)) { lo = 1; hi = 0; break; }
        uint64_t A0, A1, dB;
        pgx_rank_pair<LDS_IMAGE>(img, lds_blocks, lds_dir, lds_blow, lo, hi + 1, PGX_EXT_CV(e), 0u, A0, A1, dB);
        if (A1 == A0) { lo = 1; hi = 0; break; }
        lo = A0 + s_C[PGX_EXT_V(e)];
        hi = lo + (A1 - A0) - 1;
    }
    pgx_range r;
    r.first = lo; r.second = hi;
    out[rid] = r;
}
template __global__ void pgx_count_kernel<false>(PgxDevImage, const uint8_t *, const uint64_t *, uint64_t, pgx_range *);
template __global__ void pgx_count_kernel<true>(PgxDevImage, const uint8_t *, const uint64_t *, uint64_t, pgx_range *);

__global__ void __launch_bounds__(256)
pgx_lf_kernel(PgxDevImage img, const pgx_range *__restrict__ in, const uint8_t *__restrict__ sym, uint64_t n, pgx_range *__restrict__ out) {
    const uint64_t i = (uint64_t)blockIdx.x * blockDim.x + threadIdx.x;
    if (i >= n) return;
    const uint32_t e = img.consts->cnt_tab[sym[i]];
    pgx_range r;
    r.first = 1; r.second = 0;
    const uint64_t lo = in[i].first, hi = in[i].second;
    if (!PGX_EXT_KILL(e) && lo <= hi) {
        uint64_t A0, A1, dB;
        pgx_rank_pair<false>(img, nullptr, nullptr, nullptr, lo, hi + 1, PGX_EXT_CV(e), 0u, A0, A1, dB);
        if (A1 != A0) {
            r.first = A0 + img.consts->C[PGX_EXT_V(e)];
            r.second = r.first + (A1 - A0) - 1;
        }
    }
    out[i] = r;
}

__global__ void __launch_bounds__(256)
pgx_fmf_kernel(PgxDevImage img, const uint8_t *__restrict__ reads, const uint64_t *__restrict__ offsets, const uint64_t *__restrict__ read_of,
               const uint64_t *__restrict__ xs, uint64_t n, uint64_t min_len, uint64_t min_occ, PgxHeavyResult *__restrict__ out) {
    __shared__ uint32_t s_ext[512];
    __shared__ uint64_t s_C[8];
    pgx_stage_tables<false>(img, s_ext, s_C, nullptr, nullptr, nullptr);
// ... 55 lines not shown
```

pangenome-index_amd/csrc/pgx_runtime.hip:

```cpp
#include <dlfcn.h>

#include <string>

#include "pgx_runtime_internal.hpp"

const Roctx &roctx() {
    static const Roctx r = [] {
        Roctx x;
        const char *e = std::getenv("PGX_ROCTX");
        if (!e || !std::atoi(e)) return x;
        void *h = dlopen("librocprofiler-sdk-roctx.so", RTLD_NOW | RTLD_GLOBAL);
        if (!h) h = dlopen("libroctx64.so", RTLD_NOW | RTLD_GLOBAL);
        if (!h) return x;
        x.push = reinterpret_cast<int (*)(const char *)>(dlsym(h, "roctxRangePushA"));
        x.pop = reinterpret_cast<int (*)()>(dlsym(h, "roctxRangePop"));
        x.mark = reinterpret_cast<void (*)(const char *)>(dlsym(h, "roctxMarkA"));
        x.on = x.push && x.pop && x.mark;
        return x;
    }();
    return r;
}

int checked_device_count() {
    int n = 0;
    hipError_t e = hipGetDeviceCount(&n);
    if (e != hipSuccess || n <= 0) {
        (void)hipGetLastError();
        throw Error(PGX_ERR_NO_DEVICE, "no usable HIP device (libpgx has no CPU fallback)");
    }
    return n;
}

void use_device(int device) {
    int n = checked_device_count();
    if (device < 0 || device >= n) throw Error(PGX_ERR_ARG, "device ordinal out of range");
    HIPCHECK(hipSetDevice(device));
}

extern "C" pgx_status pgx_host_alloc(size_t bytes, void **out) {
    PGX_GUARD_BEGIN
    if (!out) throw Error(PGX_ERR_ARG, "pgx_host_alloc: null argument");
    *out = nullptr;
    (void)checked_device_count();
    void *p = nullptr;
    hipError_t e = hipHostMalloc(&p, bytes ? bytes : 1, hipHostMallocPortable);
    if (e != hipSuccess) { (void)hipGetLastError(); throw Error(PGX_ERR_NOMEM, std::string("hipHostMalloc failed: ") + hipGetErrorString(e)); }
    *out = p;
    return PGX_OK;
    PGX_GUARD_END
}
extern "C" void pgx_host_free(void *p) {
    if (p) (void)hipHostFree(p);
}

extern "C" pgx_status pgx_device_count(int *n) {
    PGX_GUARD_BEGIN
    if (!n) throw Error(PGX_ERR_ARG, "pgx_device_count: null argument");
    *n = 0;
    *n = checked_device_count();
    return PGX_OK;
    PGX_GUARD_END
}

extern "C" pgx_status pgx_device_name(int device, char *buf, size_t buflen) {
    PGX_GUARD_BEGIN
    if (!buf || !buflen) throw Error(PGX_ERR_ARG, "pgx_device_name: null argument");
    use_device(device);
    hipDeviceProp_t prop;
    HIPCHECK(hipGetDeviceProperties(&prop, device));
    std::snprintf(buf, buflen, "%s (%s, %d CUs)", prop.name, prop.gcnArchName, prop.multiProcessorCount);
    return PGX_OK;
    PGX_GUARD_END
}

void scan_excl(int mode, const void *in, uint64_t n, uint64_t min_len, uint64_t *out, DevBuf &tmp, hipStream_t s, uint64_t *total_out, const uint64_t *n_dev) {
    if (n == 0) {
        HIPCHECK(hipMemsetAsync(out, 0, 8, s));
        if (total_out) HIPCHECK(hipMemsetAsync(total_out, 0, 8, s));
        return;
    }
    static const bool three = [] { const char *e = std::getenv("PGX_SCAN_THREE"); return e && e[0] == '1'; }();
    if (!three) {
        const uint64_t nt = (n + PGX_SCAN1_TILE_ITEMS - 1) / PGX_SCAN1_TILE_ITEMS;
        tmp.ensure((nt + 2) * 8);
        if (tmp.scan_epoch == 0 || tmp.scan_epoch >= 0x3FFFFu) {
            HIPCHECK(hipMemsetAsync(tmp.p, 0, tmp.cap, s));
            tmp.scan_epoch = 0;
            if (const char *e = std::getenv("PGX_SCAN_EPOCH0")) tmp.scan_epoch = (uint32_t)std::min<unsigned long>(std::strtoul(e, nullptr, 0), 0x3FFFEul);
        }
        tmp.scan_epoch++;
        unsigned long long *st = tmp.as<unsigned long long>();
        const uint32_t ep = tmp.scan_epoch;
        switch (mode) {
        case 0: hipLaunchKernelGGL(pgx_scan_onepass_kernel<0>, dim3((unsigned)nt), dim3(256), 0, s, in, n, min_len, out, total_out, n_dev, st, ep); break;
        case 1: hipLaunchKernelGGL(pgx_scan_onepass_kernel<1>, dim3((unsigned)nt), dim3(256), 0, s, in, n, min_len, out, total_out, n_dev, st, ep); break;
        case 2: hipLaunchKernelGGL(pgx_scan_onepass_kernel<2>, dim3((unsigned)nt), dim3(256), 0, s, in, n, min_len, out, total_out, n_dev, st, ep); break;
        case 3: hipLaunchKernelGGL(pgx_scan_onepass_kernel<3>, dim3((unsigned)nt), dim3(256), 0, s, in, n, min_len, out, total_out, n_dev, st, ep); break;
        case 4: hipLaunchKernelGGL(pgx_scan_onepass_kernel<4>, dim3((unsigned)nt), dim3(256), 0, s, in, n, min_len, out, total_out, n_dev, st, ep); break;
        default: hipLaunchKernelGGL(pgx_scan_onepass_kernel<5>, dim3((unsigned)nt), dim3(256), 0, s, in, n, min_len, out, total_out, n_dev, st, ep); break;
        }
        HIPCHECK(hipGetLastError());
        return;
    }
    const uint64_t nb = (n + PGX_SCAN_BLOCK_ITEMS - 1) / PGX_SCAN_BLOCK_ITEMS;
    tmp.ensure((nb + 1) * 8);
    tmp.scan_epoch = 0;
    uint64_t *sums = tmp.as<uint64_t>();
    hipLaunchKernelGGL(pgx_scan_partial_kernel, dim3((unsigned)nb), dim3(256), 0, s, mode, in, n, min_len, sums, n_dev);
    const int raw = nb <= 2048;
    if (!raw) hipLaunchKernelGGL(pgx_scan_sums_kernel, dim3(1), dim3(256), 0, s, sums, nb);
    hipLaunchKernelGGL(pgx_scan_apply_kernel, dim3((unsigned)nb), dim3(256), 0, s, mode, in, n, min_len, (const uint64_t *)sums, nb, out, total_out, raw, n_dev);
    HIPCHECK(hipGetLastError());
}

void pgx_use_device(int device) { use_device(device); }
void pgx_scan_u64(const uint64_t *in, uint64_t n, uint64_t *out, uint64_t *tmp, hipStream_t s) {
    if (n == 0) { HIPCHECK(hipMemsetAsync(out, 0, 8, s)); return; }
    const uint64_t nb = (n + PGX_SCAN_BLOCK_ITEMS - 1) / PGX_SCAN_BLOCK_ITEMS;
    hipLaunchKernelGGL(pgx_scan_partial_kernel, dim3((unsigned)nb), dim3(256), 0, s, 1, (const void *)in, n, (uint64_t)0, tmp, (const uint64_t *)nullptr);
    const int raw = nb <= 2048;
    if (!raw) hipLaunchKernelGGL(pgx_scan_sums_kernel, dim3(1), dim3(256), 0, s, tmp, nb);
    hipLaunchKernelGGL(pgx_scan_apply_kernel, dim3((unsigned)nb), dim3(256), 0, s, 1, (const void *)in, n, (uint64_t)0, (const uint64_t *)tmp, nb, out, (uint64_t *)nullptr, raw, (const uint64_t *)nullptr);
    HIPCHECK(hipGetLastError());
}

void read_scalars(void *dst, const void *dptr, size_t bytes, hipStream_t s) {
    static thread_local void *pin = nullptr;
    if (!pin) HIPCHECK(hipHostMalloc(&pin, 512, hipHostMallocPortable));
    if (bytes > 512) throw Error(PGX_ERR_ARG, "read_scalars: too many bytes");
    HIPCHECK(hipMemcpyAsync(pin, dptr, bytes, hipMemcpyDeviceToHost, s));
    HIPCHECK(hipStreamSynchronize(s));
    std::memcpy(dst, pin, bytes);
}

extern "C" pgx_status pgx_locate_next_batch(pgx_index *h, int device, const uint64_t *prev, uint64_t n, uint64_t *out) {
    PGX_GUARD_BEGIN
    if (!h || (n && (!prev || !out))) throw Error(PGX_ERR_ARG, "pgx_locate_next_batch: null argument");
    pgx_device_image *d = locate_image(h, device);
    if (!n) return PGX_OK;
    DevBuf di, dout;
    try {
        di.ensure(n * 8); dout.ensure(n * 8);
        HIPCHECK(hipMemcpy(di.p, prev, n * 8, hipMemcpyHostToDevice));
        hipLaunchKernelGGL(pgx_locate_next_kernel, dim3(grid_for(n, 256)), dim3(256), 0, nullptr, d->loc, di.as<uint64_t>(), n,
                           dout.as<uint64_t>());
        HIPCHECK(hipGetLastError());
        HIPCHECK(hipMemcpy(out, dout.p, n * 8, hipMemcpyDeviceToHost));
    } catch (...) {
        di.release(); dout.release();
        throw;
    }
    di.release(); dout.release();
    return PGX_OK;
    PGX_GUARD_END
}

void locate_core(pgx_index *h, pgx_device_image *d, const uint64_t *first, const uint64_t *last, uint64_t n, uint32_t flags,
                 std::vector<uint64_t> &h_off, DevBuf &vals_out, uint64_t &n_vals_out) {
    const uint64_t bwt_n = d->loc.n;
    std::vector<uint64_t> cnt(n), voff(n + 1);
    voff[0] = 0;
    for (uint64_t i = 0; i < n; i++) {
        if (last[i] < first[i]) cnt[i] = 0;
        else {
            if (last[i] >= bwt_n) throw Error(PGX_ERR_ARG, "pgx_locate_batch: range " + std::to_string(i) + " ends beyond the BWT");
            cnt[i] = last[i] - first[i] + 1;
        }
        voff[i + 1] = voff[i] + cnt[i];
    }
    const uint64_t V = voff[n];
    DevBuf dqs, dqe, drun0, dnp, dpoff, dvoff, dcnt, scan_tmp, dlist, dneed, dsoff, dscratch, ducount, duoff;
    DevBuf *all[] = {&dqs, &dqe, &drun0, &dnp, &dpoff, &dvoff, &dcnt, &scan_tmp, &dlist, &dneed, &dsoff, &dscratch, &ducount, &duoff};
    DevBuf gbuf;
    try {
        hipStream_t s = nullptr;
        dqs.ensure(n * 8); dqe.ensure(n * 8); drun0.ensure(n * 8); dnp.ensure(n * 8); dpoff.ensure((n + 1) * 8); dvoff.ensure((n + 1) * 8);
        HIPCHECK(hipMemcpy(dqs.p, first, n * 8, hipMemcpyHostToDevice));
        HIPCHECK(hipMemcpy(dqe.p, last, n * 8, hipMemcpyHostToDevice));
        HIPCHECK(hipMemcpy(dvoff.p, voff.data(), (n + 1) * 8, hipMemcpyHostToDevice));
        hipLaunchKernelGGL(pgx_locate_plan_kernel, dim3(grid_for(n, 256)), dim3(256), 0, s, d->loc, dqs.as<uint64_t>(), dqe.as<uint64_t>(), n,
                           drun0.as<uint64_t>(), dnp.as<uint64_t>());
        HIPCHECK(hipGetLastError());
// ... 225 lines not shown
    PGX_GUARD_BEGIN
    if (!h || !offsets || (n && (!read_of || !x || !next_x || !mem || !has_mem))) throw Error(PGX_ERR_ARG, "pgx_find_mems_function_batch: null argument");
    if (!h->has_rank) throw Error(PGX_ERR_ARG, "pgx_find_mems_function_batch: index opened without an r-index");
    pgx_device_image *d = device_image(h, device);
    if (!n) return PGX_OK;
    for (uint64_t i = 0; i < n_reads; i++) {
        if (offsets[i + 1] < offsets[i]) throw Error(PGX_ERR_ARG, "pgx_find_mems_function_batch: offsets must be non-decreasing");
        if (offsets[i + 1] - offsets[i] >= (1ull << 31)) throw Error(PGX_ERR_UNSUPPORTED, "read longer than 2^31 bytes");
    }
    for (uint64_t i = 0; i < n; i++)
        if (read_of[i] >= n_reads) throw Error(PGX_ERR_ARG, "pgx_find_mems_function_batch: read index out of range");
    DevBuf dr, doff, dro, dx, dout;
    DevBuf *all[] = {&dr, &doff, &dro, &dx, &dout};
    try {
        const uint64_t lo = offsets[0], bytes = offsets[n_reads] - lo;
        if (bytes && !reads) throw Error(PGX_ERR_ARG, "pgx_find_mems_function_batch: null reads");
        std::vector<uint64_t> reb(n_reads + 1);
        for (uint64_t i = 0; i <= n_reads; i++) reb[i] = offsets[i] - lo;
        dr.ensure(bytes + 32); doff.ensure((n_reads + 1) * 8); dro.ensure(n * 8); dx.ensure(n * 8); dout.ensure(n * sizeof(PgxHeavyResult));
        HIPCHECK(hipMemset((uint8_t *)dr.p + bytes, 0, 32));
        if (bytes) HIPCHECK(hipMemcpy(dr.p, reads + lo, bytes, hipMemcpyHostToDevice));
        HIPCHECK(hipMemcpy(doff.p, reb.data(), (n_reads + 1) * 8, hipMemcpyHostToDevice));
        HIPCHECK(hipMemcpy(dro.p, read_of, n * 8, hipMemcpyHostToDevice));
        HIPCHECK(hipMemcpy(dx.p, x, n * 8, hipMemcpyHostToDevice));
        hipLaunchKernelGGL(pgx_fmf_kernel, dim3(grid_for(n, 256)), dim3(256), 0, 0, d->img, dr.as<uint8_t>(), doff.as<uint64_t>(), dro.as<uint64_t>(),
                           dx.as<uint64_t>(), n, min_len, min_occ, dout.as<PgxHeavyResult>());
        HIPCHECK(hipGetLastError());
        std::vector<PgxHeavyResult> res(n);
        HIPCHECK(hipMemcpy(res.data(), dout.p, n * sizeof(PgxHeavyResult), hipMemcpyDeviceToHost));
        for (uint64_t i = 0; i < n; i++) {
            next_x[i] = res[i].next_x; mem[i] = res[i].mem; has_mem[i] = (uint8_t)res[i].has_mem;
            if (n_ext) n_ext[i] = res[i].n_ext;
        }
    } catch (...) { for (DevBuf *b : all) b->release(); throw; }
    for (DevBuf *b : all) b->release();
    return PGX_OK;
    PGX_GUARD_END
}

extern "C" pgx_status pgx_lf_batch(pgx_index *h, int device, const pgx_range *in, const uint8_t *sym, uint64_t n, pgx_range *out) {
    PGX_GUARD_BEGIN
    if (!h || (n && (!in || !sym || !out))) throw Error(PGX_ERR_ARG, "pgx_lf_batch: null argument");
    if (!h->has_rank) throw Error(PGX_ERR_ARG, "pgx_lf_batch: index opened without an r-index");
    const bool lit = literal_count(h);
    pgx_device_image *d = lit ? literal_image(h, device) : device_image(h, device);
    if (!n) return PGX_OK;
    DevBuf din, dsym, dout;
    try {
        din.ensure(n * sizeof(pgx_range)); dsym.ensure(n); dout.ensure(n * sizeof(pgx_range));
        HIPCHECK(hipMemcpy(din.p, in, n * sizeof(pgx_range), hipMemcpyHostToDevice));
        HIPCHECK(hipMemcpy(dsym.p, sym, n, hipMemcpyHostToDevice));
        if (lit)
            hipLaunchKernelGGL(pgx_lit_count_kernel, dim3(grid_for(n, 256)), dim3(256), 0, 0, d->lit, (const uint8_t *)nullptr, (const uint64_t *)nullptr,
                               (const pgx_range *)din.as<pgx_range>(), (const uint8_t *)dsym.as<uint8_t>(), n, dout.as<pgx_range>());
        else
            hipLaunchKernelGGL(pgx_lf_kernel, dim3(grid_for(n, 256)), dim3(256), 0, 0, d->img, din.as<pgx_range>(), dsym.as<uint8_t>(), n, dout.as<pgx_range>());
        HIPCHECK(hipGetLastError());
        HIPCHECK(hipMemcpy(out, dout.p, n * sizeof(pgx_range), hipMemcpyDeviceToHost));
    } catch (...) { din.release(); dsym.release(); dout.release(); throw; }
    din.release(); dsym.release(); dout.release();
    return PGX_OK;
    PGX_GUARD_END
}

extern "C" pgx_status pgx_tag_query_batch(pgx_index *h, int device, const uint64_t *start, const uint64_t *end, uint64_t n,
                                          uint64_t *run_nums, uint64_t *pos_offsets, uint64_t *positions, uint64_t positions_cap,
                                          uint64_t *n_overflow) {
    PGX_GUARD_BEGIN
    if (!h || !pos_offsets || (n && (!start || !end || !run_nums))) throw Error(PGX_ERR_ARG, "pgx_tag_query_batch: null argument");
    if (!h->has_tags) throw Error(PGX_ERR_ARG, "pgx_tag_query_batch: index opened without a tag array");
    pgx_device_image *d = device_image(h, device);
    pos_offsets[0] = 0;
    if (n_overflow) *n_overflow = 0;
    if (!n) return PGX_OK;
    DevBuf ds, de, dctr;
    TagWork w;
    try {
        hipStream_t s = nullptr;
        ds.ensure(n * 8); de.ensure(n * 8); dctr.ensure(256);
        HIPCHECK(hipMemset(dctr.p, 0, 256));
        HIPCHECK(hipMemcpy(ds.p, start, n * 8, hipMemcpyHostToDevice));
        HIPCHECK(hipMemcpy(de.p, end, n * 8, hipMemcpyHostToDevice));
        unsigned long long *ctr = dctr.as<unsigned long long>();
        tag_pipeline(d->img, nullptr, ds.as<uint64_t>(), de.as<uint64_t>(), n, w, ctr, ctr + 1, s, [](int) {});
        HIPCHECK(hipMemcpy(run_nums, w.run_nums.p, n * 8, hipMemcpyDeviceToHost));
        HIPCHECK(hipMemcpy(pos_offsets, w.pos_off.p, (n + 1) * 8, hipMemcpyDeviceToHost));
        if (positions) {
            if (positions_cap < w.n_positions) throw Error(PGX_ERR_ARG, "pgx_tag_query_batch: positions_cap too small");
            if (w.n_positions) HIPCHECK(hipMemcpy(positions, w.positions.p, w.n_positions * 8, hipMemcpyDeviceToHost));
        }
        if (n_overflow) {
            unsigned long long c = 0;
            HIPCHECK(hipMemcpy(&c, dctr.p, 8, hipMemcpyDeviceToHost));
            *n_overflow = c;
        }
    } catch (...) {
        ds.release(); de.release(); dctr.release(); w.release();
        throw;
    }
    ds.release(); de.release(); dctr.release(); w.release();
    return PGX_OK;
    PGX_GUARD_END
}
```

pangenome-index_amd/csrc/pgx_runtime_internal.hpp:

```cpp
#pragma once

#include <hip/hip_runtime.h>

#include <algorithm>
#include <cstdio>
#include <cstdlib>
#include <vector>

#include "pgx_device.h"
#include "pgx_host.hpp"
#include "pgx_runtime.hpp"

#pragma GCC visibility push(hidden)

using namespace pgx;

struct Roctx {
    int (*push)(const char *) = nullptr;
    int (*pop)() = nullptr;
    void (*mark)(const char *) = nullptr;
    bool on = false;
};
const Roctx &roctx();
struct RoctxRange {
    bool on;
    explicit RoctxRange(const char *name) : on(roctx().on) { if (on) roctx().push(name); }
    ~RoctxRange() { if (on) roctx().pop(); }
    RoctxRange(const RoctxRange &) = delete;
    RoctxRange &operator=(const RoctxRange &) = delete;
};

int checked_device_count();
void use_device(int device);
void scan_excl(int mode, const void *in, uint64_t n, uint64_t min_len, uint64_t *out, DevBuf &tmp, hipStream_t s, uint64_t *total_out = nullptr,
               const uint64_t *n_dev = nullptr);
void read_scalars(void *dst, const void *dptr, size_t bytes, hipStream_t s);
inline uint64_t read_u64(const uint64_t *dptr, hipStream_t s) {
    uint64_t v = 0;
    read_scalars(&v, dptr, 8, s);
    return v;
}

struct pgx_device_image {
    int device = -1;
    PgxDevImage img{};
    DevBuf blocks, dir, blow, consts, tstart, tvals, tdir, tpair, tbucket, seed, seed_small, seed_end, exc, pairs, first_ext, sbase2, pbase;
    DevBuf rstart, rsamp, rdir, lpos, lnext, ldir;
    DevBuf lce_sa, lce_text, lce_flags, lce_lcp;
    DevBuf lce_seq_start;
    uint64_t lce_n_seq = 0;
    int lce_state = 0;
    DevBuf lit_bstart, lit_cum, lit_runs, lit_roff, lit_tabs;
    PgxLitImage lit{};
    bool has_lit = false;
    PgxLocImage loc{};
    bool has_loc = false;
    size_t lds_bytes = 0;
};

pgx_device_image *device_image(pgx_index *h, int device);
pgx_device_image *locate_image(pgx_index *h, int device);
pgx_device_image *literal_image(pgx_index *h, int device);
void ensure_lce(pgx_index *h, pgx_device_image *d);

void locate_core(pgx_index *h, pgx_device_image *d, const uint64_t *first, const uint64_t *last, uint64_t n, uint32_t flags, std::vector<uint64_t> &h_off,
                 DevBuf &vals_out, uint64_t &n_vals_out);
void locate_check_supported(const pgx_index *h, const char *who);

inline void upload(DevBuf &b, const void *src, size_t bytes) {
    b.ensure(bytes ? bytes : 16);
    if (bytes) HIPCHECK(hipMemcpy(b.p, src, bytes, hipMemcpyHostToDevice));
}

inline unsigned grid_for(uint64_t n, unsigned per_block) {
    uint64_t g = (n + per_block - 1) / per_block;
    if (g == 0) g = 1;
    if (g > 0x7FFFFFFFull) throw Error(PGX_ERR_UNSUPPORTED, "batch too large for one launch");
    return (unsigned)g;
}

struct TagWork {
    DevBuf run_nums, first_item, seg_off, gbuf, need, scratch_off, scratch, ucount, pos_off, positions, big_list, large_list, scan_tmp, dedup, dd_table,
        single, small_list;
    uint64_t n_positions = 0, n_big = 0;
    uint64_t last_G = 0, last_P = 0, last_small = 0, last_big = 0, last_large = 0, last_largest = 0, last_rep = 0, last_dup = 0;
    bool have_last = false;
    void release() {
        DevBuf *all[] = {&run_nums, &first_item, &seg_off, &gbuf, &need, &scratch_off, &scratch, &ucount, &pos_off, &positions,
                         &big_list, &large_list, &scan_tmp, &dedup, &dd_table, &single, &small_list};
        for (DevBuf *d : all) d->release();
    }
};

struct LocWork {
    DevBuf cnt, qs, qe, voff, uoff, vals, gbuf, run0, npieces, poff, seg, lists, need, soff, scratch, ucount, uloc, ctr, scan_tmp, sets;
    HostBuf h_off, h_vals;
    hipEvent_t ev[2] = {nullptr, nullptr};
    bool valid = false, resident = false;
    uint32_t flags = 0, set_words = 0;
    uint64_t n_mems = 0, n_values = 0, n_not_located = 0;
    const uint64_t *d_off = nullptr;
    float ms = 0;
    void release() {
        DevBuf *all[] = {&cnt, &qs, &qe, &voff, &uoff, &vals, &gbuf, &run0, &npieces, &poff, &seg, &lists, &need, &soff, &scratch, &ucount, &uloc, &ctr, &scan_tmp, &sets};
        for (DevBuf *d : all) d->release();
        h_off.release(); h_vals.release();
        for (auto &e : ev)
            if (e) { (void)hipEventDestroy(e); e = nullptr; }
        valid = false;
    }
};

inline uint64_t with_slack(uint64_t v) { return v + v / 4 + 64; }

template <class Rec>
void tag_pipeline(const PgxDevImage &img, const pgx_mem *d_mems, const uint64_t *d_qs, const uint64_t *d_qe, uint64_t m, TagWork &w,
                         unsigned long long *d_nover, unsigned long long *sc, hipStream_t s, Rec &&rec, bool spec = false,
                         const uint64_t *d_m = nullptr, uint64_t *d_abort = nullptr) {
    const uint64_t mm = m ? m : 1;
    w.run_nums.ensure(mm * 8);
    w.first_item.ensure(mm * 8);
    w.seg_off.ensure((m + 1) * 8);
    w.need.ensure(mm * 8);
    w.scratch_off.ensure((m + 1) * 8);
    w.ucount.ensure(mm * 8);
    w.pos_off.ensure((m + 1) * 8);
    w.big_list.ensure(mm * 8);
    w.large_list.ensure(mm * 8);
    w.single.ensure(mm * 8);
    w.small_list.ensure(mm * 8);
    const uint64_t *u_sc = reinterpret_cast<const uint64_t *>(sc);
    const uint64_t *dn_small = spec ? u_sc + 5 : nullptr, *dn_big = spec ? u_sc + 0 : nullptr, *dn_large = spec ? u_sc + 1 : nullptr;
    const uint64_t *dn_rep = spec ? u_sc + 6 : nullptr, *dn_dup = spec ? u_sc + 7 : nullptr;
    const uint64_t *ab = spec ? d_abort : nullptr;
    if (!spec) d_m = nullptr;
    auto fixed_grid = [](uint64_t n, unsigned per_block, unsigned max_blocks) { return (unsigned)std::min<uint64_t>(std::max<uint64_t>((n + per_block - 1) / per_block, 1), max_blocks); };
    if (m) {
        const unsigned g = spec ? fixed_grid(m, PGX_TAG_LOCATE_THREADS, 8192) : grid_for(m, PGX_TAG_LOCATE_THREADS);
        hipLaunchKernelGGL(pgx_tag_locate_kernel, dim3(g), dim3(PGX_TAG_LOCATE_THREADS), 0, s, img, d_mems, d_qs, d_qe, m, d_m, ab,
                           w.run_nums.as<uint64_t>(), w.first_item.as<uint64_t>(), w.need.as<uint64_t>(), w.big_list.as<uint64_t>(), w.large_list.as<uint64_t>(),
                           sc, sc + 1, w.single.as<uint64_t>(), w.ucount.as<uint64_t>(), d_nover, w.small_list.as<uint64_t>(), sc + 5);
        HIPCHECK(hipGetLastError());
    }
    scan_excl(5, w.run_nums.p, m, 0, w.seg_off.as<uint64_t>(), w.scan_tmp, s, reinterpret_cast<uint64_t *>(sc + 3), d_m);
    uint64_t G, nbig, nlarge, nsmall, largest;
    if (!spec) {
        uint64_t hv[6] = {0, 0, 0, 0, 0, 0};
        read_scalars(hv, sc, 48, s);
        G = hv[3]; nbig = hv[0]; nlarge = hv[1]; nsmall = hv[5]; largest = hv[2];
    if (std::getenv("PGX_DEBUG_COUNTERS")) std::fprintf(stderr, "[pgx] tag stage: m %llu big %llu large %llu largest %llu G %llu small %llu\n", (unsigned long long)m,
                                                            (unsigned long long)nbig, (unsigned long long)nlarge, (unsigned long long)largest, (unsigned long long)G, (unsigned long long)nsmall);
    } else {
        G = with_slack(w.last_G); nbig = with_slack(w.last_big); nlarge = with_slack(w.last_large); nsmall = with_slack(w.last_small);
        uint64_t p2 = 64;
        while (p2 < 2 * w.last_largest && p2 < PGX_SORT_WG_LDS_CAP) p2 <<= 1;
        largest = p2;
        hipLaunchKernelGGL(pgx_spec_check_kernel, dim3(1), dim3(64), 0, s, u_sc + 3, G, u_sc + 1, nlarge, u_sc + 2, largest, u_sc + 0, nbig, d_abort);
        hipLaunchKernelGGL(pgx_spec_check_kernel, dim3(1), dim3(64), 0, s, u_sc + 5, nsmall, (const uint64_t *)nullptr, (uint64_t)0, (const uint64_t *)nullptr,
                           (uint64_t)0, (const uint64_t *)nullptr, (uint64_t)0, d_abort);
        HIPCHECK(hipGetLastError());
        if (largest > PGX_SORT_WG_LDS_CAP) throw Error(PGX_ERR_ARG, "speculative tag stage with a query beyond the LDS sort capacity");
    }
    uint64_t S = 0;
    if (largest > PGX_SORT_WG_LDS_CAP) {
        scan_excl(1, w.need.p, m, 0, w.scratch_off.as<uint64_t>(), w.scan_tmp, s);
        S = read_u64(w.scratch_off.as<uint64_t>() + m, s);
    }
    w.n_big = nbig;
    rec(0);
    w.gbuf.ensure((G ? G : 1) * 8);
    w.scratch.ensure((S ? S : 1) * 8);
    if (nsmall) {
        const unsigned g = spec ? fixed_grid(nsmall, 16, 16384) : grid_for(nsmall, 16);
        hipLaunchKernelGGL(pgx_tag_small_kernel, dim3(g), dim3(256), 0, s, img, (const uint64_t *)w.small_list.as<uint64_t>(), nsmall, dn_small, ab,
                           w.run_nums.as<uint64_t>(), w.first_item.as<uint64_t>(), w.seg_off.as<uint64_t>(), w.gbuf.as<uint64_t>(),
                           w.ucount.as<uint64_t>(), d_nover);
        HIPCHECK(hipGetLastError());
    }
    rec(1);
    if (nbig) {
        const unsigned g = spec ? fixed_grid(nbig, 4, 8192) : grid_for(nbig, 4);
        hipLaunchKernelGGL(pgx_tag_gather_kernel, dim3(g), dim3(256), 0, s, img, (const uint64_t *)w.big_list.as<uint64_t>(), nbig, dn_big, ab,
                           w.run_nums.as<uint64_t>(), w.first_item.as<uint64_t>(), w.seg_off.as<uint64_t>(), w.gbuf.as<uint64_t>(), d_nover);
        hipLaunchKernelGGL(pgx_tag_sort_unique_kernel, dim3(g), dim3(256), 0, s, (const uint64_t *)w.big_list.as<uint64_t>(), nbig, dn_big, ab,
                           w.run_nums.as<uint64_t>(), w.seg_off.as<uint64_t>(), w.gbuf.as<uint64_t>(), w.ucount.as<uint64_t>());
        HIPCHECK(hipGetLastError());
    }
    uint64_t nrep = 0, ndup = 0;
    if (nlarge) {
        uint64_t p2max = 64;
        while (p2max < largest && p2max < PGX_SORT_WG_LDS_CAP) p2max <<= 1;
        const size_t lds = (size_t)p2max * 8;
        HIPCHECK(hipFuncSetAttribute((const void *)pgx_tag_sort_large_kernel, hipFuncAttributeMaxDynamicSharedMemorySize,
                                     (int)(PGX_SORT_WG_LDS_CAP * 8)));
        uint64_t tcap = 64;
        while (tcap < 2 * nlarge) tcap <<= 1;
        w.dd_table.ensure(tcap * 8);
        w.dedup.ensure(3 * nlarge * 8);
        uint64_t *d_reps = w.dedup.as<uint64_t>(), *d_pairs = d_reps + nlarge;
        HIPCHECK(hipMemsetAsync(w.dd_table.p, 0, tcap * 8, s));
        hipLaunchKernelGGL(pgx_tag_dedup_kernel, dim3(fixed_grid(nlarge, 256, 1024)), dim3(256), 0, s, (const uint64_t *)w.large_list.as<uint64_t>(), nlarge, dn_large, ab,
                           (const uint64_t *)w.first_item.as<uint64_t>(), (const uint64_t *)w.run_nums.as<uint64_t>(), w.dd_table.as<unsigned long long>(), tcap - 1,
                           d_reps, sc + 6, d_pairs, sc + 7);
        HIPCHECK(hipGetLastError());
        if (!spec) {
            uint64_t rd[2] = {0, 0};
            read_scalars(rd, sc + 6, 16, s);
            nrep = rd[0]; ndup = rd[1];
    if (std::getenv("PGX_DEBUG_COUNTERS")) std::fprintf(stderr, "[pgx] tag stage: representatives %llu duplicates %llu\n", (unsigned long long)nrep, (unsigned long long)ndup);
        } else { nrep = nlarge; ndup = nlarge; }
        if (nrep) {
            hipLaunchKernelGGL(pgx_tag_gather_kernel, dim3(spec ? fixed_grid(nrep, 4, 8192) : grid_for(nrep, 4)), dim3(256), 0, s, img, (const uint64_t *)d_reps, nrep,
                               dn_rep, ab, w.run_nums.as<uint64_t>(), w.first_item.as<uint64_t>(), w.seg_off.as<uint64_t>(), w.gbuf.as<uint64_t>(), d_nover);
            hipLaunchKernelGGL(pgx_tag_sort_large_kernel, dim3(spec ? fixed_grid(nrep, 1, 2048) : grid_for(nrep, 1)), dim3(1024), lds, s, (const uint64_t *)d_reps, nrep,
                               dn_rep, ab, w.run_nums.as<uint64_t>(), w.seg_off.as<uint64_t>(), w.gbuf.as<uint64_t>(), w.scratch.as<uint64_t>(),
                               w.scratch_off.as<uint64_t>(), w.ucount.as<uint64_t>());
        }
        if (ndup)
            hipLaunchKernelGGL(pgx_tag_copy_dups_kernel, dim3(spec ? fixed_grid(ndup, 256, 4096) : grid_for(ndup, 256)), dim3(256), 0, s, (const uint64_t *)d_pairs, ndup,
                               dn_dup, ab, img.n_tag_items, w.first_item.as<uint64_t>(), w.run_nums.as<uint64_t>(), w.seg_off.as<uint64_t>(),
                               w.gbuf.as<uint64_t>(), w.ucount.as<uint64_t>(), d_nover);
        HIPCHECK(hipGetLastError());
    }
    scan_excl(1, w.ucount.p, m, 0, w.pos_off.as<uint64_t>(), w.scan_tmp, s, reinterpret_cast<uint64_t *>(sc + 8), d_m);
    uint64_t P;
    if (!spec) {
        w.n_positions = read_u64(reinterpret_cast<const uint64_t *>(sc + 8), s);
        P = w.n_positions;
    } else {
        P = with_slack(w.last_P);
        hipLaunchKernelGGL(pgx_spec_check_kernel, dim3(1), dim3(64), 0, s, u_sc + 8, P, (const uint64_t *)nullptr, (uint64_t)0, (const uint64_t *)nullptr, (uint64_t)0,
                           (const uint64_t *)nullptr, (uint64_t)0, d_abort);
    }
    w.positions.ensure((P ? P : 1) * 8);
    if (m) {
        const uint64_t *lists[3] = {w.small_list.as<uint64_t>(), w.big_list.as<uint64_t>(), w.large_list.as<uint64_t>()};
        const uint64_t counts[3] = {nsmall, nbig, nlarge};
        const uint64_t *dcounts[3] = {dn_small, dn_big, dn_large};
        for (int li = 0; li < 3; li++)
            if (counts[li])
                hipLaunchKernelGGL(pgx_tag_compact_kernel, dim3(spec ? fixed_grid(counts[li], 16, 16384) : grid_for(counts[li], 16)), dim3(256), 0, s, lists[li], counts[li],
                                   dcounts[li], ab, w.ucount.as<uint64_t>(), w.seg_off.as<uint64_t>(), w.gbuf.as<uint64_t>(), w.pos_off.as<uint64_t>(),
                                   w.positions.as<uint64_t>(), (uint64_t)PGX_TAG_COMPACT_SMALL);
        hipLaunchKernelGGL(pgx_tag_compact_single_kernel, dim3(spec ? fixed_grid(m, 256, 16384) : grid_for(m, 256)), dim3(256), 0, s, m, d_m, ab,
                           (const uint64_t *)w.run_nums.as<uint64_t>(), (const uint64_t *)w.single.as<uint64_t>(), (const uint64_t *)w.pos_off.as<uint64_t>(),
                           w.positions.as<uint64_t>());
        if (nbig)
            hipLaunchKernelGGL(pgx_tag_compact_list_kernel, dim3(spec ? fixed_grid(nbig, 1, 4096) : grid_for(nbig, 1)), dim3(256), 0, s, (const uint64_t *)w.big_list.as<uint64_t>(), nbig,
                               dn_big, ab, w.ucount.as<uint64_t>(), w.seg_off.as<uint64_t>(), w.gbuf.as<uint64_t>(), w.pos_off.as<uint64_t>(),
                               w.positions.as<uint64_t>(), (uint64_t)PGX_TAG_COMPACT_SMALL);
        if (nlarge)
            hipLaunchKernelGGL(pgx_tag_compact_list_kernel, dim3(spec ? fixed_grid(nlarge, 1, 4096) : grid_for(nlarge, 1)), dim3(256), 0, s,
                               (const uint64_t *)w.large_list.as<uint64_t>(), nlarge, dn_large, ab, w.ucount.as<uint64_t>(), w.seg_off.as<uint64_t>(),
                               w.gbuf.as<uint64_t>(), w.pos_off.as<uint64_t>(), w.positions.as<uint64_t>(), (uint64_t)PGX_TAG_COMPACT_SMALL);
        HIPCHECK(hipGetLastError());
    }
    rec(2);
    if (!spec) {
        w.last_G = G; w.last_P = P; w.last_small = nsmall; w.last_big = nbig; w.last_large = nlarge; w.last_largest = largest;
        w.last_rep = nrep; w.last_dup = ndup;
        w.have_last = true;
    }
}

#pragma GCC visibility pop
```

pangenome-index_amd/csrc/pgx_tag_kernels.hip:

```cpp
#include <hip/hip_runtime.h>
#include <stdint.h>

#include "pgx_device.h"

#define PGX_TSTART(img, r) ((img).tpair ? (img).tpair[(r)].x : (img).tstart[(r)])
__device__ __forceinline__ uint64_t pgx_tag_rank(const PgxDevImage &img, uint64_t x) {
    const uint64_t nr = img.n_tag_runs;
    uint64_t di = x >> img.tag_dir_shift;
    if (di + 1 >= img.tag_dir_entries) return nr;
    uint64_t lo = img.tdir[di], hi = img.tdir[di + 1];
    while (lo < hi) {
        const uint64_t mid = (lo + hi) >> 1;
        if (PGX_TSTART(img, mid) <= x) lo = mid + 1; else hi = mid;
    }
    return lo;
}

__global__ void __launch_bounds__(256)
pgx_tag_bucket_kernel(const uint64_t *__restrict__ tstart, const uint64_t *__restrict__ tvals, uint64_t n_runs, uint64_t n_items, uint32_t shift,
                      uint64_t n_buckets, uint4 *__restrict__ out) {
    for (uint64_t b = (uint64_t)blockIdx.x * blockDim.x + threadIdx.x; b < n_buckets; b += (uint64_t)gridDim.x * blockDim.x) {
        const uint64_t p0 = b << shift, p1 = (b + 1) << shift;
        uint64_t lo = 0, hi = n_runs;
        while (lo < hi) { const uint64_t mid = (lo + hi) >> 1; if (tstart[mid] < p0) lo = mid + 1; else hi = mid; }
        const uint64_t r0 = lo;
        hi = n_runs;
        while (lo < hi) { const uint64_t mid = (lo + hi) >> 1; if (tstart[mid] < p1) lo = mid + 1; else hi = mid; }
        const uint64_t c = lo - r0;
        uint32_t dw[32];
#pragma unroll
        for (int i = 0; i < 32; i++) dw[i] = 0u;
        dw[0] = (uint32_t)r0;
        if (c > PGX_TBUCKET_RUNS) dw[1] = 255u;
        else {
            dw[1] = (uint32_t)c;
#pragma unroll
            for (uint32_t i = 0; i < PGX_TBUCKET_RUNS; i++)
                if (i < c) dw[2 + (i >> 1)] |= (uint32_t)(tstart[r0 + i] - p0) << (16u * (i & 1u));
#pragma unroll
            for (uint32_t i = 0; i < PGX_TBUCKET_RUNS + 2u; i++) {
                const uint64_t it = r0 + i;
                const uint64_t v = (i <= c + 1 && it >= 1 && it - 1 < n_items) ? tvals[it - 1] : 0ull;
                dw[8 + 2 * i] = (uint32_t)v; dw[9 + 2 * i] = (uint32_t)(v >> 32);
            }
        }
        uint4 *o = out + b * 8;
#pragma unroll
        for (int i = 0; i < 8; i++) o[i] = make_uint4(dw[4 * i], dw[4 * i + 1], dw[4 * i + 2], dw[4 * i + 3]);
    }
}
__device__ __forceinline__ uint32_t pgx_tbucket_le(const uint4 &h0, const uint4 &h1, uint32_t c, uint32_t off) {
    const uint32_t w[5] = {h0.z, h0.w, h1.x, h1.y, h1.z};
    uint32_t k = 0;
#pragma unroll
    for (uint32_t i = 0; i < PGX_TBUCKET_RUNS; i++) {
        const uint32_t s = (w[i >> 1] >> (16u * (i & 1u))) & 0xFFFFu;
        k += (i < c && s <= off) ? 1u : 0u;
    }
    return k;
}

#define PGX_DEV_COUNT(n, n_dev) ((n_dev) ? ((*(n_dev)) < (n) ? (*(n_dev)) : (n)) : (n))
#define PGX_ABORTED(abort) ((abort) && *(abort))

__global__ void __launch_bounds__(PGX_TAG_LOCATE_THREADS)
pgx_tag_locate_kernel(PgxDevImage img, const pgx_mem *__restrict__ mems, const uint64_t *__restrict__ qstart,
                      const uint64_t *__restrict__ qend, uint64_t n_cap, const uint64_t *__restrict__ n_dev, const uint64_t *__restrict__ abort,
                      uint64_t *__restrict__ run_nums,
                      uint64_t *__restrict__ first_item, uint64_t *__restrict__ need, uint64_t *__restrict__ big_list, uint64_t *__restrict__ large_list,
                      unsigned long long *__restrict__ n_big, unsigned long long *__restrict__ n_large, uint64_t *__restrict__ single,
                      uint64_t *__restrict__ ucount, unsigned long long *__restrict__ n_overflow, uint64_t *__restrict__ small_list,
                      unsigned long long *__restrict__ n_small) {
  if (PGX_ABORTED(abort)) return;
  const uint64_t n = PGX_DEV_COUNT(n_cap, n_dev);
  __shared__ uint32_t s_cnt[PGX_TAG_LOCATE_THREADS / 64];
  __shared__ unsigned long long s_base;
  for (uint64_t base = (uint64_t)blockIdx.x * blockDim.x; base < n; base += (uint64_t)gridDim.x * blockDim.x) {
    const uint64_t i = base + threadIdx.x;
    const bool valid = i < n;
    uint64_t cnt = 0;
    if (valid) {
        uint64_t st, en;
        if (mems) { st = mems[i].bwt_start; en = st + (uint64_t)mems[i].size - 1; }
        else { st = qstart[i]; en = qend[i]; }
        bool done = false;
        uint64_t f = 0, g = 0, bval = 0;
        bool bval_ok = false;
        if (img.tbucket && en >= st && (st >> img.tbucket_shift) < img.n_tbuckets) {
            const uint32_t sh = img.tbucket_shift, msk = (1u << sh) - 1u;
            const uint64_t b0 = st >> sh, b1 = en >> sh;
            const uint4 *bp = img.tbucket + b0 * 8;
            const uint4 h0 = bp[0], h1 = bp[1];
            const uint32_t c0 = h0.y & 0xFFu;
            if (c0 != 255u) {
                f = (uint64_t)h0.x + pgx_tbucket_le(h0, h1, c0, (uint32_t)st & msk);
                if (b1 == b0) { g = (uint64_t)h0.x + pgx_tbucket_le(h0, h1, c0, (uint32_t)en & msk); done = true; }
                else if (b1 < img.n_tbuckets) {
                    const uint4 *ep = img.tbucket + b1 * 8;
                    const uint4 e0 = ep[0], e1 = ep[1];
                    const uint32_t c1 = e0.y & 0xFFu;
                    if (c1 != 255u) { g = (uint64_t)e0.x + pgx_tbucket_le(e0, e1, c1, (uint32_t)en & msk); done = true; }
                }
                if (done && g == f) {
                    const uint64_t fi0 = (f % 10) ? f - 1 : f;
                    const uint32_t slot = (uint32_t)(fi0 + 1 - (uint64_t)h0.x);
                    const uint2 *vp = reinterpret_cast<const uint2 *>(bp) + 4 + slot;
                    const uint2 vv = *vp;
                    bval = (uint64_t)vv.x | ((uint64_t)vv.y << 32);
                    bval_ok = true;
                }
            }
        }
        if (!done) {
        f = pgx_tag_rank(img, st);
        g = f;
        if (en >= st) {
            const uint64_t nr = img.n_tag_runs;
            uint64_t step = 1, lo = f, hi = f;
            while (hi < nr && PGX_TSTART(img, hi) <= en) { lo = hi + 1; hi = (hi + step < nr) ? hi + step : nr; step <<= 1; }
            while (lo < hi) {
                const uint64_t mid = (lo + hi) >> 1;
                if (PGX_TSTART(img, mid) <= en) lo = mid + 1; else hi = mid;
            }
            g = lo;
        } else g = pgx_tag_rank(img, en);
        }
        cnt = g - f + 1;
        run_nums[i] = cnt;
        const uint64_t fi = (f % 10) ? f - 1 : f;
        first_item[i] = fi;
        if (cnt == 1) {
            uint64_t v = 0;
            if (fi < img.n_tag_items) v = bval_ok ? bval : (img.tpair ? img.tpair[fi].y : img.tvals[fi]);
            else atomicAdd(n_overflow, 1ull);
            single[i] = v;
            ucount[i] = 1;
        } else if (cnt == 0) ucount[i] = 0;
        uint64_t p2 = 64;
        while (p2 < cnt && p2 < (1ull << 62)) p2 <<= 1;
        need[i] = p2 > PGX_SORT_WG_LDS_CAP ? p2 : 0;
        if (cnt > PGX_SORT_LDS_CAP) {
            large_list[atomicAdd(n_large, 1ull)] = i;
            atomicMax(n_large + 1, (unsigned long long)cnt);
        }
        else if (cnt > PGX_TAG_SMALL) big_list[atomicAdd(n_big, 1ull)] = i;
    }
    const bool is_small = valid && cnt >= 2 && cnt <= PGX_TAG_SMALL;
    const unsigned long long m = __ballot(is_small);
    const int lane = threadIdx.x & 63, wv = threadIdx.x >> 6;
    if (lane == 0) s_cnt[wv] = (uint32_t)__popcll(m);
    __syncthreads();
    if (threadIdx.x == 0) {
        uint32_t tot = 0;
        for (int k = 0; k < PGX_TAG_LOCATE_THREADS / 64; k++) { const uint32_t c = s_cnt[k]; s_cnt[k] = tot; tot += c; }
        s_base = tot ? atomicAdd(n_small, (unsigned long long)tot) : 0ull;
    }
    __syncthreads();
    if (is_small) small_list[s_base + s_cnt[wv] + (unsigned long long)__popcll(m & ((1ull << lane) - 1ull))] = i;
    __syncthreads();
  }
}

__global__ void __launch_bounds__(256)
pgx_tag_small_kernel(PgxDevImage img, const uint64_t *__restrict__ list, uint64_t n_cap, const uint64_t *__restrict__ n_dev,
                     const uint64_t *__restrict__ abort, const uint64_t *__restrict__ run_nums,
                     const uint64_t *__restrict__ first_item, const uint64_t *__restrict__ seg_off, uint64_t *__restrict__ buf,
                     uint64_t *__restrict__ ucount, unsigned long long *__restrict__ n_overflow) {
  if (PGX_ABORTED(abort)) return;
  const uint64_t n = PGX_DEV_COUNT(n_cap, n_dev);
  const int lane = threadIdx.x & 63, l16 = lane & 15, grp = lane >> 4;
  for (uint64_t wbase = ((uint64_t)blockIdx.x * blockDim.x + (threadIdx.x & ~63u)) >> 4; wbase < n; wbase += ((uint64_t)gridDim.x * blockDim.x) >> 4) {
    const uint64_t w16 = wbase + (uint64_t)grp;
    const bool valid = w16 < n;
    const uint64_t q = valid ? list[w16] : 0;
    const uint64_t cnt = valid ? run_nums[q] : 0;
    const bool mine = valid;
    uint64_t v = ~0ull;
    bool over = false;
    if (mine && (uint64_t)l16 < cnt) {
        const uint64_t it = first_item[q] + (uint64_t)l16;
        if (it < img.n_tag_items) v = img.tvals[it];
        else { v = 0; over = true; }
    }
#pragma unroll
    for (int k = 2; k <= 16; k <<= 1) {
#pragma unroll
        for (int jj = k >> 1; jj > 0; jj >>= 1) {
            const uint64_t o = __shfl_xor(v, jj, 64);
            const bool up = ((l16 & k) == 0), lower = ((l16 & jj) == 0);
            const uint64_t mn = v < o ? v : o, mx = v < o ? o : v;
            v = (lower == up) ? mn : mx;
        }
    }
    const uint64_t prev = __shfl_up(v, 1, 64);
    const bool keep = mine && (uint64_t)l16 < cnt && (l16 == 0 || v != prev);
    const unsigned long long mask = __ballot(keep);
    const unsigned long long omask = __ballot(over);
    const uint32_t gm = (uint32_t)(mask >> (16 * grp)) & 0xFFFFu;
    if (keep) buf[seg_off[q] + (uint64_t)__popc(gm & ((1u << l16) - 1u))] = v;
    if (mine && l16 == 0) {
        ucount[q] = (uint64_t)__popc(gm);
        if ((omask >> (16 * grp)) & 0xFFFFull) atomicAdd(n_overflow, 1ull);
    }
  }
}

__global__ void __launch_bounds__(256)
pgx_tag_gather_kernel(PgxDevImage img, const uint64_t *__restrict__ list, uint64_t n_cap, const uint64_t *__restrict__ n_dev,
                      const uint64_t *__restrict__ abort, const uint64_t *__restrict__ run_nums,
                      const uint64_t *__restrict__ first_item, const uint64_t *__restrict__ seg_off, uint64_t *__restrict__ buf,
                      unsigned long long *__restrict__ n_overflow) {
  if (PGX_ABORTED(abort)) return;
  const uint64_t n_list = PGX_DEV_COUNT(n_cap, n_dev);
  const int lane = threadIdx.x & 63;
  for (uint64_t w = ((uint64_t)blockIdx.x * blockDim.x + threadIdx.x) >> 6; w < n_list; w += ((uint64_t)gridDim.x * blockDim.x) >> 6) {
    const uint64_t q = list[w];
    const uint64_t cnt = run_nums[q], src = first_item[q], dst = seg_off[q];
    bool over = false;
    for (uint64_t t = lane; t < cnt; t += 64) {
        const uint64_t it = src + t;
        uint64_t v = 0;
        if (it < img.n_tag_items) v = img.tvals[it]; else over = true;
        buf[dst + t] = v;
    }
    if (__any(over) && lane == 0) atomicAdd(n_overflow, 1ull);
  }
}

template <class Ptr>
__device__ __forceinline__ uint64_t pgx_wave_sort_unique(Ptr arr, uint64_t *__restrict__ seg, uint64_t cnt, uint64_t p2, int lane) {
    for (uint64_t t = lane; t < p2; t += 64) arr[t] = t < cnt ? seg[t] : ~0ull;
    __threadfence_block();
    __builtin_amdgcn_wave_barrier();
    for (uint64_t k = 2; k <= p2; k <<= 1) {
        for (uint64_t jj = k >> 1; jj > 0; jj >>= 1) {
            for (uint64_t t = lane; t < p2 / 2; t += 64) {
                const uint64_t lo_i = ((t & ~(jj - 1)) << 1) | (t & (jj - 1));
                const uint64_t hi_i = lo_i | jj;
                const uint64_t a = arr[lo_i], b = arr[hi_i];
                const bool up = ((lo_i & k) == 0);
                if ((a > b) == up) { arr[lo_i] = b; arr[hi_i] = a; }
            }
// ... 242 lines not shown
```

Measured before the change: 1.105 billion.

## Fuse MEM compaction with tag locate and scatter singles during scan

Adds a fused compact+locate kernel that, for single-chunk batches with tags, gathers each read's MEMs from slots and immediately runs tag location, replacing the separate compact kernel. The tag locate step is restructured to compute segment offsets in-block via wave prefix sums, and new scan modes (6, 7) let the one-pass scan compute sort needs and place single-occurrence positions directly. The aim is to remove kernel launches and intermediate passes over the MEM array. The cost is a per-MEM binary search over read offsets in shared memory, extra capacity and abort checks, and more complex control paths.

```diff
diff --git a/pangenome-index_amd/csrc/pgx_batch.hip b/pangenome-index_amd/csrc/pgx_batch.hip
--- a/pangenome-index_amd/csrc/pgx_batch.hip
+++ b/pangenome-index_amd/csrc/pgx_batch.hip
@@ -349,6 +349,7 @@
     bool has_side_heavy_ext;
     uint32_t side_heavy_ext;
     bool debug_counters;
+    int post_fused;
     bool fm_stats;
 };
 
@@ -373,6 +374,7 @@
     if (const char *e = std::getenv("PGX_FM_HEAVY_EXT")) k.heavy_ext = (uint32_t)std::strtoul(e, nullptr, 10);
     if (const char *e = std::getenv("PGX_FM_SIDE_HEAVY_EXT")) { k.has_side_heavy_ext = true; k.side_heavy_ext = (uint32_t)std::strtoul(e, nullptr, 10); }
     k.debug_counters = is_set("PGX_DEBUG_COUNTERS");
+    k.post_fused = post_fused_knob();
     k.fm_stats = is_set("PGX_FM_STATS");
     return k;
 }
@@ -459,6 +461,8 @@
     bool want_tags;
     unsigned long long *ctr = nullptr;
     bool spec = false, arena_on = false;
+    bool fused = false;
+    TagSlots tslots{};
     uint64_t cm_cap = 0;
     const void *kfn = nullptr, *kfn_wide = nullptr, *kfn_pairs = nullptr;
     uint32_t kfn_bits = 0, kfn_pairs_bits = 0;
@@ -739,6 +743,12 @@
     hipStream_t s = r.s;
     const uint64_t cn = c.r1 - c.r0;
     b->mems.ensure_keep((mem_base + cm ? mem_base + cm : 1) * sizeof(pgx_mem), mem_base * sizeof(pgx_mem));
+    if (r.fused) {
+        r.tslots = TagSlots{c.r0, cn, c.slot_base, r.spec ? r.cm_cap : ~0ull, ovf_cap, b->slot_off.as<uint64_t>(), (const uint64_t *)(b->mem_off.as<uint64_t>() + c.r0),
+                            b->slots.as<pgx_mem>(), (const uint32_t *)(b->ovf_base.as<uint32_t>() - c.r0)};
+        record(b, 3, s);
+        return;
+    }
     hipLaunchKernelGGL(pgx_compact_mems_kernel, dim3(grid_for(cn, 256)), dim3(256), 0, s, c.r0, cn, b->slot_off.as<uint64_t>(),
                        c.slot_base, b->slots.as<pgx_mem>(), b->mem_count.as<uint32_t>(), (const uint64_t *)(b->mem_off.as<uint64_t>() + c.r0), mem_base,
                        b->mems.as<pgx_mem>(), r.spec ? r.cm_cap : ~0ull, reinterpret_cast<uint64_t *>(r.ctr + PGX_CTR_ABORT),
@@ -847,6 +857,7 @@
     r.spec = may_speculate && chunks.size() == 1 && b->shape_valid && b->shape_reads == r.n && b->shape_min_len == r.min_len && b->shape_min_occ == r.min_occ &&
              b->shape_tags == r.want_tags && (!r.want_tags || (b->tw.have_last && b->tw.last_largest <= PGX_SORT_WG_LDS_CAP)) && r.k.spec && !r.k.force_redo;
     r.cm_cap = with_slack(b->last_mems);
+    r.fused = chunks.size() == 1 && r.want_tags && r.k.post_fused != 0;
     uint64_t mem_base = 0;
     for (size_t ci = 0; ci < chunks.size(); ci++) {
         record(b, 1, s);
@@ -867,8 +878,12 @@
     }
     record(b, 3, s);
     if (r.want_tags) {
+        TagOptions opt;
+        opt.post_fused = r.k.post_fused;
+        opt.debug_counters = r.k.debug_counters;
+        opt.slots = r.fused ? &r.tslots : nullptr;
         tag_pipeline(r.img, b->mems.as<pgx_mem>(), nullptr, nullptr, b->n_mems, b->tw, r.ctr + PGX_CTR_TAG_OVERFLOW, r.ctr + PGX_CTR_TAG0, s,
-                     [&](int stage) { record(b, 4 + stage, s); }, r.spec, reinterpret_cast<const uint64_t *>(r.ctr + PGX_CTR_MEMS),
+                     [&](int stage) { record(b, 4 + stage, s); }, opt, r.spec, reinterpret_cast<const uint64_t *>(r.ctr + PGX_CTR_MEMS),
                      reinterpret_cast<uint64_t *>(r.ctr + PGX_CTR_ABORT));
         b->n_positions = b->tw.n_positions;
         b->ran_tags = true;
diff --git a/pangenome-index_amd/csrc/pgx_device.h b/pangenome-index_amd/csrc/pgx_device.h
--- a/pangenome-index_amd/csrc/pgx_device.h
+++ b/pangenome-index_amd/csrc/pgx_device.h
@@ -140,15 +140,25 @@
                                uint64_t min_len, uint64_t min_occ, PgxHeavyResult *out);
 __global__ void pgx_lf_kernel(PgxDevImage img, const pgx_range *in, const uint8_t *sym, uint64_t n, pgx_range *out);
 __global__ void pgx_scan_partial_kernel(int mode, const void *in, uint64_t n, uint64_t min_len, uint64_t *block_sums, const uint64_t *n_dev);
+struct PgxScanSingles {
+    const uint64_t *single;
+    uint64_t *positions;
+    uint64_t cap;
+    uint64_t *abort;
+};
 template <int MODE>
 __global__ void pgx_scan_onepass_kernel(const void *in, uint64_t n, uint64_t min_len, uint64_t *out, uint64_t *total_out, const uint64_t *n_dev,
-                                        unsigned long long *state, uint32_t epoch);
+                                        unsigned long long *state, uint32_t epoch, PgxScanSingles singles);
 __global__ void pgx_scan_sums_kernel(uint64_t *block_sums, uint64_t nb);
 __global__ void pgx_scan_apply_kernel(int mode, const void *in, uint64_t n, uint64_t min_len, const uint64_t *block_sums,
                                       uint64_t nb, uint64_t *out, uint64_t *total_out, int raw_sums, const uint64_t *n_dev);
 __global__ void pgx_compact_mems_kernel(uint64_t first_read, uint64_t n_reads, const uint64_t *slot_off, uint64_t slot_base,
                                         const pgx_mem *slots, const uint32_t *mem_count, const uint64_t *local_off,
                                         uint64_t mem_base, pgx_mem *mems, uint64_t cap_mems, uint64_t *abort, const uint32_t *ovf_base, uint64_t ovf_cap);
+#define PGX_FAST_SLOTS 4u
+__device__ __forceinline__ uint64_t pgx_slot_index(uint64_t read_in_chunk, uint64_t chunk_reads, uint64_t slot, uint32_t nm) {
+    return nm < PGX_FAST_SLOTS ? (uint64_t)nm * chunk_reads + read_in_chunk : chunk_reads * PGX_FAST_SLOTS + slot + nm;
+}
 __global__ void pgx_tag_pair_kernel(const uint64_t *tstart, const uint64_t *tvals, uint64_t n_runs, uint64_t n_items, ulonglong2 *out);
 __global__ void pgx_tag_bucket_kernel(const uint64_t *tstart, const uint64_t *tvals, uint64_t n_runs, uint64_t n_items, uint32_t shift, uint64_t n_buckets, uint4 *out);
 #define PGX_TAG_LOCATE_THREADS 1024
@@ -156,10 +166,21 @@
 #define PGX_TAG_SMALL 16
 #define PGX_SORT_WG_LDS_CAP 16384
 
+struct PgxTagLocateOut {
+    uint64_t *run_nums, *first_item, *seg_off, *single, *ucount;
+    uint64_t *small_list, *big_list, *large_list;
+    unsigned long long *sc;
+    unsigned long long *n_overflow;
+    uint64_t *abort;
+    uint64_t cap_gathered;
+    uint64_t cap_small, cap_big, cap_large, cap_largest;
+    uint32_t segments;
+};
 __global__ void pgx_tag_locate_kernel(PgxDevImage img, const pgx_mem *mems, const uint64_t *qstart, const uint64_t *qend,
-                                      uint64_t n, const uint64_t *n_dev, const uint64_t *abort, uint64_t *run_nums, uint64_t *first_item, uint64_t *need,
-                                      uint64_t *big_list, uint64_t *large_list, unsigned long long *n_big, unsigned long long *n_large, uint64_t *single,
-                                      uint64_t *ucount, unsigned long long *n_overflow, uint64_t *small_list, unsigned long long *n_small);
+                                      uint64_t n, const uint64_t *n_dev, PgxTagLocateOut out);
+__global__ void pgx_compact_locate_kernel(PgxDevImage img, uint64_t first_read, uint64_t n_reads, const uint64_t *slot_off, uint64_t slot_base,
+                                          const pgx_mem *slots, const uint64_t *local_off, pgx_mem *mems, uint64_t cap_mems,
+                                          const uint32_t *ovf_base, uint64_t ovf_cap, PgxTagLocateOut out);
 __global__ void pgx_tag_small_kernel(PgxDevImage img, const uint64_t *list, uint64_t n, const uint64_t *n_dev, const uint64_t *abort, const uint64_t *run_nums,
                                      const uint64_t *first_item, const uint64_t *seg_off, uint64_t *buf, uint64_t *ucount, unsigned long long *n_overflow);
 __global__ void pgx_tag_gather_kernel(PgxDevImage img, const uint64_t *list, uint64_t n_list, const uint64_t *n_dev, const uint64_t *abort,
diff --git a/pangenome-index_amd/csrc/pgx_kernels.hip b/pangenome-index_amd/csrc/pgx_kernels.hip
--- a/pangenome-index_amd/csrc/pgx_kernels.hip
+++ b/pangenome-index_amd/csrc/pgx_kernels.hip
@@ -465,14 +465,10 @@
   }
 }
 
-#define PGX_FAST_SLOTS 4u
 #ifndef PGX_PAIRS_PACKED_WAVES
 #define PGX_PAIRS_PACKED_WAVES 5
 #endif
 #define PGX_PK_GROUP 12u
-__device__ __forceinline__ uint64_t pgx_slot_index(uint64_t read_in_chunk, uint64_t chunk_reads, uint64_t slot, uint32_t nm) {
-    return nm < PGX_FAST_SLOTS ? (uint64_t)nm * chunk_reads + read_in_chunk : chunk_reads * PGX_FAST_SLOTS + slot + nm;
-}
 __device__ __forceinline__ uint64_t pgx_slot_extent(const uint64_t *__restrict__ slot_off, uint64_t slot_base, uint32_t *__restrict__ ovf_base, uint64_t ovf_cap,
                                                     unsigned long long *__restrict__ ctr, uint64_t rid, uint32_t nm, int32_t len, int32_t x, uint64_t min_len) {
     if (!ovf_cap) return slot_off[rid] - slot_base;
@@ -1746,10 +1742,17 @@
 
 __device__ __forceinline__ uint64_t pgx_scan_load(int mode, const void *in, uint64_t i, uint64_t min_len) {
     if (mode == 0) return ((const uint32_t *)in)[i];
-    if (mode == 1) return ((const uint64_t *)in)[i];
+    if (mode == 1 || mode == 7) return ((const uint64_t *)in)[i];
     if (mode == 3) return ((const uint8_t *)in)[i] == (uint8_t)min_len ? 1u : 0u;
     if (mode == 4) return ((const uint8_t *)in)[i];
     if (mode == 5) { const uint64_t v = ((const uint64_t *)in)[i]; return v == 1 ? 0 : v; }
+    if (mode == 6) {
+        const uint64_t v = ((const uint64_t *)in)[i];
+        if (v <= PGX_SORT_WG_LDS_CAP) return 0;
+        uint64_t p2 = 2 * (uint64_t)PGX_SORT_WG_LDS_CAP;
+        while (p2 < v && p2 < (1ull << 62)) p2 <<= 1;
+        return p2;
+    }
     const uint64_t *off = (const uint64_t *)in;
     const uint64_t len = off[i + 1] - off[i];
     if (len < min_len) return 0;
@@ -1853,7 +1856,7 @@
 template <int MODE>
 __global__ void __launch_bounds__(256)
 pgx_scan_onepass_kernel(const void *in, uint64_t n_cap, uint64_t min_len, uint64_t *__restrict__ out, uint64_t *__restrict__ total_out,
-                        const uint64_t *__restrict__ n_dev, unsigned long long *__restrict__ state, uint32_t epoch) {
+                        const uint64_t *__restrict__ n_dev, unsigned long long *__restrict__ state, uint32_t epoch, PgxScanSingles singles) {
     constexpr int mode = MODE;
     __shared__ uint64_t s_wave[4];
     __shared__ uint64_t s_prefix;
@@ -1870,10 +1873,17 @@
     const int lane = threadIdx.x & 63, w = threadIdx.x >> 6;
     const uint64_t b0 = (uint64_t)tile * (256u * PGX_SCAN1_ROUNDS) + (uint64_t)w * (64u * PGX_SCAN1_ROUNDS);
     uint64_t x[PGX_SCAN1_ROUNDS], carry = 0;
+    uint32_t ones = 0;
 #pragma unroll
     for (int r = 0; r < PGX_SCAN1_ROUNDS; r++) {
         const uint64_t i = b0 + (uint64_t)(r * 64 + lane);
         x[r] = i < n ? pgx_scan_load(mode, in, i, min_len) : 0;
+        if (MODE == 7) ones |= (x[r] == 1 ? 1u : 0u) << r;
+    }
+    uint64_t sv[MODE == 7 ? PGX_SCAN1_ROUNDS : 1];
+    if (MODE == 7) {
+#pragma unroll
+        for (int r = 0; r < PGX_SCAN1_ROUNDS; r++) sv[r] = (ones >> r) & 1u ? singles.single[b0 + (uint64_t)(r * 64 + lane)] : 0;
     }
 #pragma unroll
     for (int r = 0; r < PGX_SCAN1_ROUNDS; r++) {
@@ -1936,19 +1946,22 @@
     for (int r = 0; r < PGX_SCAN1_ROUNDS; r++) {
         const uint64_t i = b0 + (uint64_t)(r * 64 + lane);
         if (i < n) out[i] = P + x[r];
+        if (MODE == 7 && ((ones >> r) & 1u) && P + x[r] < singles.cap) singles.positions[P + x[r]] = sv[MODE == 7 ? r : 0];
     }
     if (tile == last_tile && threadIdx.x == 0) {
         const uint64_t grand = s_prefix + tile_total;
         out[n] = grand;
         if (total_out) *total_out = grand;
+        if (MODE == 7 && singles.abort && grand > singles.cap) atomicOr((unsigned long long *)singles.abort, 1ull);
     }
     if (tile == gridDim.x - 1 && threadIdx.x == 0)
         __hip_atomic_store(reinterpret_cast<uint32_t *>(state), 0u, __ATOMIC_RELAXED, __HIP_MEMORY_SCOPE_AGENT);
 }
 
 #define PGX_SCAN1_INSTANTIATE(M) \
-    template __global__ void pgx_scan_onepass_kernel<M>(const void *, uint64_t, uint64_t, uint64_t *, uint64_t *, const uint64_t *, unsigned long long *, uint32_t);
+    template __global__ void pgx_scan_onepass_kernel<M>(const void *, uint64_t, uint64_t, uint64_t *, uint64_t *, const uint64_t *, unsigned long long *, uint32_t, PgxScanSingles);
 PGX_SCAN1_INSTANTIATE(0) PGX_SCAN1_INSTANTIATE(1) PGX_SCAN1_INSTANTIATE(2) PGX_SCAN1_INSTANTIATE(3) PGX_SCAN1_INSTANTIATE(4) PGX_SCAN1_INSTANTIATE(5)
+PGX_SCAN1_INSTANTIATE(6) PGX_SCAN1_INSTANTIATE(7)
 
 __global__ void __launch_bounds__(256)
 pgx_compact_mems_kernel(uint64_t first_read, uint64_t n_reads, const uint64_t *__restrict__ slot_off, uint64_t slot_base,
diff --git a/pangenome-index_amd/csrc/pgx_runtime.hip b/pangenome-index_amd/csrc/pgx_runtime.hip
--- a/pangenome-index_amd/csrc/pgx_runtime.hip
+++ b/pangenome-index_amd/csrc/pgx_runtime.hip
@@ -73,13 +73,22 @@
     PGX_GUARD_END
 }
 
-void scan_excl(int mode, const void *in, uint64_t n, uint64_t min_len, uint64_t *out, DevBuf &tmp, hipStream_t s, uint64_t *total_out, const uint64_t *n_dev) {
+static bool scan_three() {
+    static const bool three = [] { const char *e = std::getenv("PGX_SCAN_THREE"); return e && e[0] == '1'; }();
+    return three;
+}
+bool scan_is_onepass() { return !scan_three(); }
+
+void scan_excl(int mode, const void *in, uint64_t n, uint64_t min_len, uint64_t *out, DevBuf &tmp, hipStream_t s, uint64_t *total_out, const uint64_t *n_dev,
+               const PgxScanSingles *singles) {
+    if (mode == 7 && (!singles || scan_three())) throw Error(PGX_ERR_ARG, "scan_excl: mode 7 is the one-pass kernel's, with the positions it places");
     if (n == 0) {
         HIPCHECK(hipMemsetAsync(out, 0, 8, s));
         if (total_out) HIPCHECK(hipMemsetAsync(total_out, 0, 8, s));
         return;
     }
-    static const bool three = [] { const char *e = std::getenv("PGX_SCAN_THREE"); return e && e[0] == '1'; }();
+    const bool three = scan_three();
+    const PgxScanSingles sg = singles ? *singles : PgxScanSingles{};
     if (!three) {
         const uint64_t nt = (n + PGX_SCAN1_TILE_ITEMS - 1) / PGX_SCAN1_TILE_ITEMS;
         tmp.ensure((nt + 2) * 8);
@@ -92,12 +101,15 @@
         unsigned long long *st = tmp.as<unsigned long long>();
         const uint32_t ep = tmp.scan_epoch;
         switch (mode) {
-        case 0: hipLaunchKernelGGL(pgx_scan_onepass_kernel<0>, dim3((unsigned)nt), dim3(256), 0, s, in, n, min_len, out, total_out, n_dev, st, ep); break;
-        case 1: hipLaunchKernelGGL(pgx_scan_onepass_kernel<1>, dim3((unsigned)nt), dim3(256), 0, s, in, n, min_len, out, total_out, n_dev, st, ep); break;
-        case 2: hipLaunchKernelGGL(pgx_scan_onepass_kernel<2>, dim3((unsigned)nt), dim3(256), 0, s, in, n, min_len, out, total_out, n_dev, st, ep); break;
-        case 3: hipLaunchKernelGGL(pgx_scan_onepass_kernel<3>, dim3((unsigned)nt), dim3(256), 0, s, in, n, min_len, out, total_out, n_dev, st, ep); break;
-        case 4: hipLaunchKernelGGL(pgx_scan_onepass_kernel<4>, dim3((unsigned)nt), dim3(256), 0, s, in, n, min_len, out, total_out, n_dev, st, ep); break;
-        default: hipLaunchKernelGGL(pgx_scan_onepass_kernel<5>, dim3((unsigned)nt), dim3(256), 0, s, in, n, min_len, out, total_out, n_dev, st, ep); break;
+        case 0: hipLaunchKernelGGL(pgx_scan_onepass_kernel<0>, dim3((unsigned)nt), dim3(256), 0, s, in, n, min_len, out, total_out, n_dev, st, ep, sg); break;
+        case 1: hipLaunchKernelGGL(pgx_scan_onepass_kernel<1>, dim3((unsigned)nt), dim3(256), 0, s, in, n, min_len, out, total_out, n_dev, st, ep, sg); break;
+        case 2: hipLaunchKernelGGL(pgx_scan_onepass_kernel<2>, dim3((unsigned)nt), dim3(256), 0, s, in, n, min_len, out, total_out, n_dev, st, ep, sg); break;
+        case 3: hipLaunchKernelGGL(pgx_scan_onepass_kernel<3>, dim3((unsigned)nt), dim3(256), 0, s, in, n, min_len, out, total_out, n_dev, st, ep, sg); break;
+        case 4: hipLaunchKernelGGL(pgx_scan_onepass_kernel<4>, dim3((unsigned)nt), dim3(256), 0, s, in, n, min_len, out, total_out, n_dev, st, ep, sg); break;
+        case 5: hipLaunchKernelGGL(pgx_scan_onepass_kernel<5>, dim3((unsigned)nt), dim3(256), 0, s, in, n, min_len, out, total_out, n_dev, st, ep, sg); break;
+        case 6: hipLaunchKernelGGL(pgx_scan_onepass_kernel<6>, dim3((unsigned)nt), dim3(256), 0, s, in, n, min_len, out, total_out, n_dev, st, ep, sg); break;
+        case 7: hipLaunchKernelGGL(pgx_scan_onepass_kernel<7>, dim3((unsigned)nt), dim3(256), 0, s, in, n, min_len, out, total_out, n_dev, st, ep, sg); break;
+        default: throw Error(PGX_ERR_ARG, "scan_excl: no such mode");
         }
         HIPCHECK(hipGetLastError());
         return;
@@ -489,7 +501,10 @@
         HIPCHECK(hipMemcpy(ds.p, start, n * 8, hipMemcpyHostToDevice));
         HIPCHECK(hipMemcpy(de.p, end, n * 8, hipMemcpyHostToDevice));
         unsigned long long *ctr = dctr.as<unsigned long long>();
-        tag_pipeline(d->img, nullptr, ds.as<uint64_t>(), de.as<uint64_t>(), n, w, ctr, ctr + 1, s, [](int) {});
+        TagOptions opt;
+        opt.post_fused = post_fused_knob();
+        opt.debug_counters = std::getenv("PGX_DEBUG_COUNTERS") != nullptr;
+        tag_pipeline(d->img, nullptr, ds.as<uint64_t>(), de.as<uint64_t>(), n, w, ctr, ctr + 1, s, [](int) {}, opt);
         HIPCHECK(hipMemcpy(run_nums, w.run_nums.p, n * 8, hipMemcpyDeviceToHost));
         HIPCHECK(hipMemcpy(pos_offsets, w.pos_off.p, (n + 1) * 8, hipMemcpyDeviceToHost));
         if (positions) {
diff --git a/pangenome-index_amd/csrc/pgx_runtime_internal.hpp b/pangenome-index_amd/csrc/pgx_runtime_internal.hpp
--- a/pangenome-index_amd/csrc/pgx_runtime_internal.hpp
+++ b/pangenome-index_amd/csrc/pgx_runtime_internal.hpp
@@ -33,7 +33,8 @@
 int checked_device_count();
 void use_device(int device);
 void scan_excl(int mode, const void *in, uint64_t n, uint64_t min_len, uint64_t *out, DevBuf &tmp, hipStream_t s, uint64_t *total_out = nullptr,
-               const uint64_t *n_dev = nullptr);
+               const uint64_t *n_dev = nullptr, const PgxScanSingles *singles = nullptr);
+bool scan_is_onepass();
 void read_scalars(void *dst, const void *dptr, size_t bytes, hipStream_t s);
 inline uint64_t read_u64(const uint64_t *dptr, hipStream_t s) {
     uint64_t v = 0;
@@ -80,13 +81,13 @@
 }
 
 struct TagWork {
-    DevBuf run_nums, first_item, seg_off, gbuf, need, scratch_off, scratch, ucount, pos_off, positions, big_list, large_list, scan_tmp, dedup, dd_table,
+    DevBuf run_nums, first_item, seg_off, gbuf, scratch_off, scratch, ucount, pos_off, positions, big_list, large_list, scan_tmp, dedup, dd_table,
         single, small_list;
     uint64_t n_positions = 0, n_big = 0;
     uint64_t last_G = 0, last_P = 0, last_small = 0, last_big = 0, last_large = 0, last_largest = 0, last_rep = 0, last_dup = 0;
     bool have_last = false;
     void release() {
-        DevBuf *all[] = {&run_nums, &first_item, &seg_off, &gbuf, &need, &scratch_off, &scratch, &ucount, &pos_off, &positions,
+        DevBuf *all[] = {&run_nums, &first_item, &seg_off, &gbuf, &scratch_off, &scratch, &ucount, &pos_off, &positions,
                          &big_list, &large_list, &scan_tmp, &dedup, &dd_table, &single, &small_list};
         for (DevBuf *d : all) d->release();
     }
@@ -113,15 +114,31 @@
 
 inline uint64_t with_slack(uint64_t v) { return v + v / 4 + 64; }
 
+inline int post_fused_knob() {
+    const char *e = std::getenv("PGX_POST_FUSED");
+    return !e ? 1 : e[0] == '0' ? 0 : e[0] == '2' ? 2 : 1;
+}
+struct TagSlots {
+    uint64_t first_read, n_reads, slot_base, cap_mems, ovf_cap;
+    const uint64_t *slot_off, *local_off;
+    const pgx_mem *slots;
+    const uint32_t *ovf_base;
+};
+struct TagOptions {
+    int post_fused = 1;
+    bool debug_counters = false;
+    const TagSlots *slots = nullptr;
+};
+
 template <class Rec>
 void tag_pipeline(const PgxDevImage &img, const pgx_mem *d_mems, const uint64_t *d_qs, const uint64_t *d_qe, uint64_t m, TagWork &w,
-                         unsigned long long *d_nover, unsigned long long *sc, hipStream_t s, Rec &&rec, bool spec = false,
+                         unsigned long long *d_nover, unsigned long long *sc, hipStream_t s, Rec &&rec, const TagOptions &opt = TagOptions(), bool spec = false,
                          const uint64_t *d_m = nullptr, uint64_t *d_abort = nullptr) {
     const uint64_t mm = m ? m : 1;
+    const bool legacy = opt.post_fused == 0;
     w.run_nums.ensure(mm * 8);
     w.first_item.ensure(mm * 8);
     w.seg_off.ensure((m + 1) * 8);
-    w.need.ensure(mm * 8);
     w.scratch_off.ensure((m + 1) * 8);
     w.ucount.ensure(mm * 8);
     w.pos_off.ensure((m + 1) * 8);
@@ -135,35 +152,55 @@
     const uint64_t *ab = spec ? d_abort : nullptr;
     if (!spec) d_m = nullptr;
     auto fixed_grid = [](uint64_t n, unsigned per_block, unsigned max_blocks) { return (unsigned)std::min<uint64_t>(std::max<uint64_t>((n + per_block - 1) / per_block, 1), max_blocks); };
-    if (m) {
+    uint64_t G = 0, nbig = 0, nlarge = 0, nsmall = 0, largest = 0;
+    if (spec) {
+        G = with_slack(w.last_G); nbig = with_slack(w.last_big); nlarge = with_slack(w.last_large); nsmall = with_slack(w.last_small);
+        uint64_t p2 = 64;
+        while (p2 < 2 * w.last_largest && p2 < PGX_SORT_WG_LDS_CAP) p2 <<= 1;
+        largest = p2;
+    }
+    PgxTagLocateOut lo{};
+    lo.run_nums = w.run_nums.as<uint64_t>(); lo.first_item = w.first_item.as<uint64_t>(); lo.seg_off = w.seg_off.as<uint64_t>();
+    lo.single = w.single.as<uint64_t>(); lo.ucount = w.ucount.as<uint64_t>();
+    lo.small_list = w.small_list.as<uint64_t>(); lo.big_list = w.big_list.as<uint64_t>(); lo.large_list = w.large_list.as<uint64_t>();
+    lo.sc = sc; lo.n_overflow = d_nover;
+    lo.abort = spec ? d_abort : nullptr;
+    lo.cap_gathered = lo.cap_small = lo.cap_big = lo.cap_large = lo.cap_largest = ~0ull;
+    if (spec && !legacy) { lo.cap_gathered = G; lo.cap_small = nsmall; lo.cap_big = nbig; lo.cap_large = nlarge; lo.cap_largest = largest; }
+    lo.segments = legacy ? 0u : 1u;
+    if (m && opt.slots && !legacy) {
+        const TagSlots &ts = *opt.slots;
+        hipLaunchKernelGGL(pgx_compact_locate_kernel, dim3(grid_for(ts.n_reads, PGX_TAG_LOCATE_THREADS)), dim3(PGX_TAG_LOCATE_THREADS), 0, s, img, ts.first_read,
+                           ts.n_reads, ts.slot_off, ts.slot_base, ts.slots, ts.local_off, const_cast<pgx_mem *>(d_mems), ts.cap_mems, ts.ovf_base, ts.ovf_cap, lo);
+        HIPCHECK(hipGetLastError());
+    } else if (m) {
         const unsigned g = spec ? fixed_grid(m, PGX_TAG_LOCATE_THREADS, 8192) : grid_for(m, PGX_TAG_LOCATE_THREADS);
-        hipLaunchKernelGGL(pgx_tag_locate_kernel, dim3(g), dim3(PGX_TAG_LOCATE_THREADS), 0, s, img, d_mems, d_qs, d_qe, m, d_m, ab,
-                           w.run_nums.as<uint64_t>(), w.first_item.as<uint64_t>(), w.need.as<uint64_t>(), w.big_list.as<uint64_t>(), w.large_list.as<uint64_t>(),
-                           sc, sc + 1, w.single.as<uint64_t>(), w.ucount.as<uint64_t>(), d_nover, w.small_list.as<uint64_t>(), sc + 5);
-        HIPCHECK(hipGetLastError());
-    }
-    scan_excl(5, w.run_nums.p, m, 0, w.seg_off.as<uint64_t>(), w.scan_tmp, s, reinterpret_cast<uint64_t *>(sc + 3), d_m);
-    uint64_t G, nbig, nlarge, nsmall, largest;
+        hipLaunchKernelGGL(pgx_tag_locate_kernel, dim3(g), dim3(PGX_TAG_LOCATE_THREADS), 0, s, img, d_mems, d_qs, d_qe, m, d_m, lo);
+        HIPCHECK(hipGetLastError());
+    }
+    if (opt.debug_counters)
+        std::fprintf(stderr, "[pgx] tag stage: first kernel %s, segments by %s\n", m && opt.slots && !legacy ? "pgx_compact_locate_kernel" : "pgx_tag_locate_kernel",
+                     legacy ? "scan" : "atomics");
+    if (legacy) scan_excl(5, w.run_nums.p, m, 0, w.seg_off.as<uint64_t>(), w.scan_tmp, s, reinterpret_cast<uint64_t *>(sc + 3), d_m);
     if (!spec) {
         uint64_t hv[6] = {0, 0, 0, 0, 0, 0};
         read_scalars(hv, sc, 48, s);
         G = hv[3]; nbig = hv[0]; nlarge = hv[1]; nsmall = hv[5]; largest = hv[2];
-    if (std::getenv("PGX_DEBUG_COUNTERS")) std::fprintf(stderr, "[pgx] tag stage: m %llu big %llu large %llu largest %llu G %llu small %llu\n", (unsigned long long)m,
-                                                            (unsigned long long)nbig, (unsigned long long)nlarge, (unsigned long long)largest, (unsigned long long)G, (unsigned long long)nsmall);
+        if (opt.debug_counters)
+            std::fprintf(stderr, "[pgx] tag stage: m %llu big %llu large %llu largest %llu G %llu small %llu\n", (unsigned long long)m, (unsigned long long)nbig,
+                         (unsigned long long)nlarge, (unsigned long long)largest, (unsigned long long)G, (unsigned long long)nsmall);
     } else {
-        G = with_slack(w.last_G); nbig = with_slack(w.last_big); nlarge = with_slack(w.last_large); nsmall = with_slack(w.last_small);
-        uint64_t p2 = 64;
-        while (p2 < 2 * w.last_largest && p2 < PGX_SORT_WG_LDS_CAP) p2 <<= 1;
-        largest = p2;
-        hipLaunchKernelGGL(pgx_spec_check_kernel, dim3(1), dim3(64), 0, s, u_sc + 3, G, u_sc + 1, nlarge, u_sc + 2, largest, u_sc + 0, nbig, d_abort);
-        hipLaunchKernelGGL(pgx_spec_check_kernel, dim3(1), dim3(64), 0, s, u_sc + 5, nsmall, (const uint64_t *)nullptr, (uint64_t)0, (const uint64_t *)nullptr,
-                           (uint64_t)0, (const uint64_t *)nullptr, (uint64_t)0, d_abort);
-        HIPCHECK(hipGetLastError());
+        if (legacy) {
+            hipLaunchKernelGGL(pgx_spec_check_kernel, dim3(1), dim3(64), 0, s, u_sc + 3, G, u_sc + 1, nlarge, u_sc + 2, largest, u_sc + 0, nbig, d_abort);
+            hipLaunchKernelGGL(pgx_spec_check_kernel, dim3(1), dim3(64), 0, s, u_sc + 5, nsmall, (const uint64_t *)nullptr, (uint64_t)0, (const uint64_t *)nullptr,
+                               (uint64_t)0, (const uint64_t *)nullptr, (uint64_t)0, d_abort);
+            HIPCHECK(hipGetLastError());
+        }
         if (largest > PGX_SORT_WG_LDS_CAP) throw Error(PGX_ERR_ARG, "speculative tag stage with a query beyond the LDS sort capacity");
     }
     uint64_t S = 0;
     if (largest > PGX_SORT_WG_LDS_CAP) {
-        scan_excl(1, w.need.p, m, 0, w.scratch_off.as<uint64_t>(), w.scan_tmp, s);
+        scan_excl(6, w.run_nums.p, m, 0, w.scratch_off.as<uint64_t>(), w.scan_tmp, s);
         S = read_u64(w.scratch_off.as<uint64_t>() + m, s);
     }
     w.n_big = nbig;
@@ -207,7 +244,7 @@
             uint64_t rd[2] = {0, 0};
             read_scalars(rd, sc + 6, 16, s);
             nrep = rd[0]; ndup = rd[1];
-    if (std::getenv("PGX_DEBUG_COUNTERS")) std::fprintf(stderr, "[pgx] tag stage: representatives %llu duplicates %llu\n", (unsigned long long)nrep, (unsigned long long)ndup);
+            if (opt.debug_counters) std::fprintf(stderr, "[pgx] tag stage: representatives %llu duplicates %llu\n", (unsigned long long)nrep, (unsigned long long)ndup);
         } else { nrep = nlarge; ndup = nlarge; }
         if (nrep) {
             hipLaunchKernelGGL(pgx_tag_gather_kernel, dim3(spec ? fixed_grid(nrep, 4, 8192) : grid_for(nrep, 4)), dim3(256), 0, s, img, (const uint64_t *)d_reps, nrep,
@@ -222,17 +259,26 @@
                                w.gbuf.as<uint64_t>(), w.ucount.as<uint64_t>(), d_nover);
         HIPCHECK(hipGetLastError());
     }
-    scan_excl(1, w.ucount.p, m, 0, w.pos_off.as<uint64_t>(), w.scan_tmp, s, reinterpret_cast<uint64_t *>(sc + 8), d_m);
+    const bool singles_in_scan = opt.post_fused == 1 && scan_is_onepass();
     uint64_t P;
-    if (!spec) {
-        w.n_positions = read_u64(reinterpret_cast<const uint64_t *>(sc + 8), s);
-        P = w.n_positions;
+    if (singles_in_scan) {
+        P = spec ? with_slack(w.last_P) : (m - std::min(m, nsmall + nbig + nlarge)) + G;
+        w.positions.ensure((P ? P : 1) * 8);
+        const PgxScanSingles sg{w.single.as<uint64_t>(), w.positions.as<uint64_t>(), P, spec ? d_abort : nullptr};
+        scan_excl(7, w.ucount.p, m, 0, w.pos_off.as<uint64_t>(), w.scan_tmp, s, reinterpret_cast<uint64_t *>(sc + 8), d_m, &sg);
+        if (!spec) w.n_positions = read_u64(reinterpret_cast<const uint64_t *>(sc + 8), s);
     } else {
-        P = with_slack(w.last_P);
-        hipLaunchKernelGGL(pgx_spec_check_kernel, dim3(1), dim3(64), 0, s, u_sc + 8, P, (const uint64_t *)nullptr, (uint64_t)0, (const uint64_t *)nullptr, (uint64_t)0,
-                           (const uint64_t *)nullptr, (uint64_t)0, d_abort);
-    }
-    w.positions.ensure((P ? P : 1) * 8);
+        scan_excl(1, w.ucount.p, m, 0, w.pos_off.as<uint64_t>(), w.scan_tmp, s, reinterpret_cast<uint64_t *>(sc + 8), d_m);
+        if (!spec) {
+            w.n_positions = read_u64(reinterpret_cast<const uint64_t *>(sc + 8), s);
+            P = w.n_positions;
+        } else {
+            P = with_slack(w.last_P);
+            hipLaunchKernelGGL(pgx_spec_check_kernel, dim3(1), dim3(64), 0, s, u_sc + 8, P, (const uint64_t *)nullptr, (uint64_t)0, (const uint64_t *)nullptr, (uint64_t)0,
+                               (const uint64_t *)nullptr, (uint64_t)0, d_abort);
+        }
+        w.positions.ensure((P ? P : 1) * 8);
+    }
     if (m) {
         const uint64_t *lists[3] = {w.small_list.as<uint64_t>(), w.big_list.as<uint64_t>(), w.large_list.as<uint64_t>()};
         const uint64_t counts[3] = {nsmall, nbig, nlarge};
@@ -242,9 +288,10 @@
                 hipLaunchKernelGGL(pgx_tag_compact_kernel, dim3(spec ? fixed_grid(counts[li], 16, 16384) : grid_for(counts[li], 16)), dim3(256), 0, s, lists[li], counts[li],
                                    dcounts[li], ab, w.ucount.as<uint64_t>(), w.seg_off.as<uint64_t>(), w.gbuf.as<uint64_t>(), w.pos_off.as<uint64_t>(),
                                    w.positions.as<uint64_t>(), (uint64_t)PGX_TAG_COMPACT_SMALL);
-        hipLaunchKernelGGL(pgx_tag_compact_single_kernel, dim3(spec ? fixed_grid(m, 256, 16384) : grid_for(m, 256)), dim3(256), 0, s, m, d_m, ab,
-                           (const uint64_t *)w.run_nums.as<uint64_t>(), (const uint64_t *)w.single.as<uint64_t>(), (const uint64_t *)w.pos_off.as<uint64_t>(),
-                           w.positions.as<uint64_t>());
+        if (!singles_in_scan)
+            hipLaunchKernelGGL(pgx_tag_compact_single_kernel, dim3(spec ? fixed_grid(m, 256, 16384) : grid_for(m, 256)), dim3(256), 0, s, m, d_m, ab,
+                               (const uint64_t *)w.run_nums.as<uint64_t>(), (const uint64_t *)w.single.as<uint64_t>(), (const uint64_t *)w.pos_off.as<uint64_t>(),
+                               w.positions.as<uint64_t>());
         if (nbig)
             hipLaunchKernelGGL(pgx_tag_compact_list_kernel, dim3(spec ? fixed_grid(nbig, 1, 4096) : grid_for(nbig, 1)), dim3(256), 0, s, (const uint64_t *)w.big_list.as<uint64_t>(), nbig,
                                dn_big, ab, w.ucount.as<uint64_t>(), w.seg_off.as<uint64_t>(), w.gbuf.as<uint64_t>(), w.pos_off.as<uint64_t>(),
@@ -257,7 +304,7 @@
     }
     rec(2);
     if (!spec) {
-        w.last_G = G; w.last_P = P; w.last_small = nsmall; w.last_big = nbig; w.last_large = nlarge; w.last_largest = largest;
+        w.last_G = G; w.last_P = w.n_positions; w.last_small = nsmall; w.last_big = nbig; w.last_large = nlarge; w.last_largest = largest;
         w.last_rep = nrep; w.last_dup = ndup;
         w.have_last = true;
     }
diff --git a/pangenome-index_amd/csrc/pgx_tag_kernels.hip b/pangenome-index_amd/csrc/pgx_tag_kernels.hip
--- a/pangenome-index_amd/csrc/pgx_tag_kernels.hip
+++ b/pangenome-index_amd/csrc/pgx_tag_kernels.hip
@@ -63,55 +63,36 @@
 #define PGX_DEV_COUNT(n, n_dev) ((n_dev) ? ((*(n_dev)) < (n) ? (*(n_dev)) : (n)) : (n))
 #define PGX_ABORTED(abort) ((abort) && *(abort))
 
-__global__ void __launch_bounds__(PGX_TAG_LOCATE_THREADS)
-pgx_tag_locate_kernel(PgxDevImage img, const pgx_mem *__restrict__ mems, const uint64_t *__restrict__ qstart,
-                      const uint64_t *__restrict__ qend, uint64_t n_cap, const uint64_t *__restrict__ n_dev, const uint64_t *__restrict__ abort,
-                      uint64_t *__restrict__ run_nums,
-                      uint64_t *__restrict__ first_item, uint64_t *__restrict__ need, uint64_t *__restrict__ big_list, uint64_t *__restrict__ large_list,
-                      unsigned long long *__restrict__ n_big, unsigned long long *__restrict__ n_large, uint64_t *__restrict__ single,
-                      uint64_t *__restrict__ ucount, unsigned long long *__restrict__ n_overflow, uint64_t *__restrict__ small_list,
-                      unsigned long long *__restrict__ n_small) {
-  if (PGX_ABORTED(abort)) return;
-  const uint64_t n = PGX_DEV_COUNT(n_cap, n_dev);
-  __shared__ uint32_t s_cnt[PGX_TAG_LOCATE_THREADS / 64];
-  __shared__ unsigned long long s_base;
-  for (uint64_t base = (uint64_t)blockIdx.x * blockDim.x; base < n; base += (uint64_t)gridDim.x * blockDim.x) {
-    const uint64_t i = base + threadIdx.x;
-    const bool valid = i < n;
-    uint64_t cnt = 0;
-    if (valid) {
-        uint64_t st, en;
-        if (mems) { st = mems[i].bwt_start; en = st + (uint64_t)mems[i].size - 1; }
-        else { st = qstart[i]; en = qend[i]; }
-        bool done = false;
-        uint64_t f = 0, g = 0, bval = 0;
-        bool bval_ok = false;
-        if (img.tbucket && en >= st && (st >> img.tbucket_shift) < img.n_tbuckets) {
-            const uint32_t sh = img.tbucket_shift, msk = (1u << sh) - 1u;
-            const uint64_t b0 = st >> sh, b1 = en >> sh;
-            const uint4 *bp = img.tbucket + b0 * 8;
-            const uint4 h0 = bp[0], h1 = bp[1];
-            const uint32_t c0 = h0.y & 0xFFu;
-            if (c0 != 255u) {
-                f = (uint64_t)h0.x + pgx_tbucket_le(h0, h1, c0, (uint32_t)st & msk);
-                if (b1 == b0) { g = (uint64_t)h0.x + pgx_tbucket_le(h0, h1, c0, (uint32_t)en & msk); done = true; }
-                else if (b1 < img.n_tbuckets) {
-                    const uint4 *ep = img.tbucket + b1 * 8;
-                    const uint4 e0 = ep[0], e1 = ep[1];
-                    const uint32_t c1 = e0.y & 0xFFu;
-                    if (c1 != 255u) { g = (uint64_t)e0.x + pgx_tbucket_le(e0, e1, c1, (uint32_t)en & msk); done = true; }
-                }
-                if (done && g == f) {
-                    const uint64_t fi0 = (f % 10) ? f - 1 : f;
-                    const uint32_t slot = (uint32_t)(fi0 + 1 - (uint64_t)h0.x);
-                    const uint2 *vp = reinterpret_cast<const uint2 *>(bp) + 4 + slot;
-                    const uint2 vv = *vp;
-                    bval = (uint64_t)vv.x | ((uint64_t)vv.y << 32);
-                    bval_ok = true;
-                }
-            }
-        }
-        if (!done) {
+__device__ __forceinline__ uint64_t pgx_tag_locate_one(const PgxDevImage &img, uint64_t st, uint64_t en, uint64_t i, const PgxTagLocateOut &o) {
+    bool done = false;
+    uint64_t f = 0, g = 0, bval = 0;
+    bool bval_ok = false;
+    if (img.tbucket && en >= st && (st >> img.tbucket_shift) < img.n_tbuckets) {
+        const uint32_t sh = img.tbucket_shift, msk = (1u << sh) - 1u;
+        const uint64_t b0 = st >> sh, b1 = en >> sh;
+        const uint4 *bp = img.tbucket + b0 * 8;
+        const uint4 h0 = bp[0], h1 = bp[1];
+        const uint32_t c0 = h0.y & 0xFFu;
+        if (c0 != 255u) {
+            f = (uint64_t)h0.x + pgx_tbucket_le(h0, h1, c0, (uint32_t)st & msk);
+            if (b1 == b0) { g = (uint64_t)h0.x + pgx_tbucket_le(h0, h1, c0, (uint32_t)en & msk); done = true; }
+            else if (b1 < img.n_tbuckets) {
+                const uint4 *ep = img.tbucket + b1 * 8;
+                const uint4 e0 = ep[0], e1 = ep[1];
+                const uint32_t c1 = e0.y & 0xFFu;
+                if (c1 != 255u) { g = (uint64_t)e0.x + pgx_tbucket_le(e0, e1, c1, (uint32_t)en & msk); done = true; }
+            }
+            if (done && g == f) {
+                const uint64_t fi0 = (f % 10) ? f - 1 : f;
+                const uint32_t slot = (uint32_t)(fi0 + 1 - (uint64_t)h0.x);
+                const uint2 *vp = reinterpret_cast<const uint2 *>(bp) + 4 + slot;
+                const uint2 vv = *vp;
+                bval = (uint64_t)vv.x | ((uint64_t)vv.y << 32);
+                bval_ok = true;
+            }
+        }
+    }
+    if (!done) {
         f = pgx_tag_rank(img, st);
         g = f;
         if (en >= st) {
@@ -124,40 +105,134 @@
             }
             g = lo;
         } else g = pgx_tag_rank(img, en);
-        }
-        cnt = g - f + 1;
-        run_nums[i] = cnt;
-        const uint64_t fi = (f % 10) ? f - 1 : f;
-        first_item[i] = fi;
-        if (cnt == 1) {
-            uint64_t v = 0;
-            if (fi < img.n_tag_items) v = bval_ok ? bval : (img.tpair ? img.tpair[fi].y : img.tvals[fi]);
-            else atomicAdd(n_overflow, 1ull);
-            single[i] = v;
-            ucount[i] = 1;
-        } else if (cnt == 0) ucount[i] = 0;
-        uint64_t p2 = 64;
-        while (p2 < cnt && p2 < (1ull << 62)) p2 <<= 1;
-        need[i] = p2 > PGX_SORT_WG_LDS_CAP ? p2 : 0;
-        if (cnt > PGX_SORT_LDS_CAP) {
-            large_list[atomicAdd(n_large, 1ull)] = i;
-            atomicMax(n_large + 1, (unsigned long long)cnt);
-        }
-        else if (cnt > PGX_TAG_SMALL) big_list[atomicAdd(n_big, 1ull)] = i;
-    }
+    }
+    const uint64_t cnt = g - f + 1;
+    o.run_nums[i] = cnt;
+    const uint64_t fi = (f % 10) ? f - 1 : f;
+    if (cnt == 1) {
+        uint64_t v = 0;
+        if (fi < img.n_tag_items) v = bval_ok ? bval : (img.tpair ? img.tpair[fi].y : img.tvals[fi]);
+        else atomicAdd(o.n_overflow, 1ull);
+        o.single[i] = v;
+        o.ucount[i] = 1;
+    } else if (cnt == 0) o.ucount[i] = 0;
+    else {
+        o.first_item[i] = fi;
+        o.single[i] = 0;
+    }
+    if (cnt > PGX_SORT_LDS_CAP) {
+        const unsigned long long at = atomicAdd(o.sc + 1, 1ull);
+        o.large_list[at] = i;
+        atomicMax(o.sc + 2, (unsigned long long)cnt);
+        if (at >= o.cap_large) atomicOr((unsigned long long *)o.abort, 2ull);
+        if (cnt > o.cap_largest) atomicOr((unsigned long long *)o.abort, 4ull);
+    } else if (cnt > PGX_TAG_SMALL) {
+        const unsigned long long at = atomicAdd(o.sc + 0, 1ull);
+        o.big_list[at] = i;
+        if (at >= o.cap_big) atomicOr((unsigned long long *)o.abort, 8ull);
+    }
+    return cnt;
+}
+
+struct PgxTagLocateShared {
+    uint32_t cnt[PGX_TAG_LOCATE_THREADS / 64];
+    unsigned long long seg[PGX_TAG_LOCATE_THREADS / 64];
+    unsigned long long base_small, base_seg;
+    uint32_t seg_ok;
+};
+__device__ __forceinline__ void pgx_tag_locate_lists(bool valid, uint64_t cnt, uint64_t i, const PgxTagLocateOut &o, PgxTagLocateShared &sh) {
     const bool is_small = valid && cnt >= 2 && cnt <= PGX_TAG_SMALL;
     const unsigned long long m = __ballot(is_small);
     const int lane = threadIdx.x & 63, wv = threadIdx.x >> 6;
-    if (lane == 0) s_cnt[wv] = (uint32_t)__popcll(m);
+    const uint64_t want = (o.segments && valid && cnt >= 2) ? cnt : 0;
+    uint64_t inc = want;
+    if (o.segments && __ballot(want != 0)) {
+#pragma unroll
+        for (int off = 1; off < 64; off <<= 1) {
+            const uint64_t t = __shfl_up(inc, off, 64);
+            if (lane >= off) inc += t;
+        }
+    }
+    if (lane == 0) sh.cnt[wv] = (uint32_t)__popcll(m);
+    if (lane == 63) sh.seg[wv] = inc;
     __syncthreads();
     if (threadIdx.x == 0) {
         uint32_t tot = 0;
-        for (int k = 0; k < PGX_TAG_LOCATE_THREADS / 64; k++) { const uint32_t c = s_cnt[k]; s_cnt[k] = tot; tot += c; }
-        s_base = tot ? atomicAdd(n_small, (unsigned long long)tot) : 0ull;
+        unsigned long long gtot = 0;
+        for (int k = 0; k < PGX_TAG_LOCATE_THREADS / 64; k++) {
+            const uint32_t c = sh.cnt[k]; sh.cnt[k] = tot; tot += c;
+            const unsigned long long g = sh.seg[k]; sh.seg[k] = gtot; gtot += g;
+        }
+        sh.base_small = tot ? atomicAdd(o.sc + 5, (unsigned long long)tot) : 0ull;
+        if (tot && sh.base_small + tot > o.cap_small) atomicOr((unsigned long long *)o.abort, 1ull);
+        sh.base_seg = gtot ? atomicAdd(o.sc + 3, gtot) : 0ull;
+        sh.seg_ok = 1u;
+        if (gtot && sh.base_seg + gtot > o.cap_gathered) {
+            atomicOr((unsigned long long *)o.abort, 1ull);
+            sh.seg_ok = 0u;
+        }
     }
     __syncthreads();
-    if (is_small) small_list[s_base + s_cnt[wv] + (unsigned long long)__popcll(m & ((1ull << lane) - 1ull))] = i;
+    if (is_small) o.small_list[sh.base_small + sh.cnt[wv] + (unsigned long long)__popcll(m & ((1ull << lane) - 1ull))] = i;
+    if (want && sh.seg_ok) o.seg_off[i] = sh.base_seg + sh.seg[wv] + (inc - want);
     __syncthreads();
+}
+
+__global__ void __launch_bounds__(PGX_TAG_LOCATE_THREADS)
+pgx_tag_locate_kernel(PgxDevImage img, const pgx_mem *__restrict__ mems, const uint64_t *__restrict__ qstart,
+                      const uint64_t *__restrict__ qend, uint64_t n_cap, const uint64_t *__restrict__ n_dev, PgxTagLocateOut o) {
+  if (PGX_ABORTED(o.abort)) return;
+  const uint64_t n = PGX_DEV_COUNT(n_cap, n_dev);
+  __shared__ PgxTagLocateShared sh;
+  for (uint64_t base = (uint64_t)blockIdx.x * blockDim.x; base < n; base += (uint64_t)gridDim.x * blockDim.x) {
+    const uint64_t i = base + threadIdx.x;
+    const bool valid = i < n;
+    uint64_t cnt = 0;
+    if (valid) {
+        uint64_t st, en;
+        if (mems) { st = mems[i].bwt_start; en = st + (uint64_t)mems[i].size - 1; }
+        else { st = qstart[i]; en = qend[i]; }
+        cnt = pgx_tag_locate_one(img, st, en, i, o);
+    }
+    pgx_tag_locate_lists(valid, cnt, i, o, sh);
+  }
+}
+
+__global__ void __launch_bounds__(PGX_TAG_LOCATE_THREADS)
+pgx_compact_locate_kernel(PgxDevImage img, uint64_t first_read, uint64_t n_reads, const uint64_t *__restrict__ slot_off, uint64_t slot_base,
+                          const pgx_mem *__restrict__ slots, const uint64_t *__restrict__ local_off, pgx_mem *__restrict__ mems, uint64_t cap_mems,
+                          const uint32_t *__restrict__ ovf_base, uint64_t ovf_cap, PgxTagLocateOut o) {
+  if (PGX_ABORTED(o.abort)) return;
+  __shared__ PgxTagLocateShared sh;
+  __shared__ uint64_t s_off[PGX_TAG_LOCATE_THREADS + 1];
+  const uint64_t t0 = (uint64_t)blockIdx.x * PGX_TAG_LOCATE_THREADS;
+  if (t0 >= n_reads) return;
+  const uint32_t nr = (uint32_t)(n_reads - t0 < PGX_TAG_LOCATE_THREADS ? n_reads - t0 : PGX_TAG_LOCATE_THREADS);
+  for (uint32_t t = threadIdx.x; t <= nr; t += PGX_TAG_LOCATE_THREADS) s_off[t] = local_off[t0 + t];
+  __syncthreads();
+  const uint64_t m0 = s_off[0], m1 = s_off[nr];
+  if (m1 > cap_mems) {
+      if (m1 > m0 && o.abort && threadIdx.x == 0) atomicOr((unsigned long long *)o.abort, 16ull);
+      return;
+  }
+  for (uint64_t base = m0; base < m1; base += PGX_TAG_LOCATE_THREADS) {
+    const uint64_t i = base + threadIdx.x;
+    const bool valid = i < m1;
+    uint64_t cnt = 0;
+    if (valid) {
+        uint32_t lo = 0, hi = nr;
+        while (hi - lo > 1) {
+            const uint32_t mid = (lo + hi) >> 1;
+            if (s_off[mid] <= i) lo = mid; else hi = mid;
+        }
+        const uint64_t t = t0 + lo, rid = first_read + t;
+        const uint32_t k = (uint32_t)(i - s_off[lo]);
+        const uint64_t src = k < PGX_FAST_SLOTS ? 0ull : (ovf_cap ? (uint64_t)ovf_base[rid] - PGX_FAST_SLOTS : slot_off[rid] - slot_base);
+        const pgx_mem mem = slots[pgx_slot_index(t, n_reads, src, k)];
+        mems[i] = mem;
+        cnt = pgx_tag_locate_one(img, mem.bwt_start, mem.bwt_start + (uint64_t)mem.size - 1, i, o);
+    }
+    pgx_tag_locate_lists(valid, cnt, i, o, sh);
   }
 }
 
```

New measurement: 1.153 billion (median of 6 runs). 1.04x the previous value.
